# skyzh/tiny-llm

Hardware: AMD Instinct MI355X
Metric: Qwen3-4B int4 decode tokens/sec/GPU; achieved HBM GB/s vs roofline (higher is better)
Workload: dtype bf16; 1 GPU; Qwen3-4B int4 single-prompt KV-cache decode (BASELINE.json configs[1]); decode_steps=2003, batch_per_gpu=1, parallelism=request-parallel x1 (no collective on the data path), page_size=128, graph_replay=True, prefill_step=128, replay_route=aql

## Files before the change

include/tinyllm_engine.h:

```cpp
#ifndef TINYLLM_ENGINE_H
#define TINYLLM_ENGINE_H

#include <stddef.h>
#include <stdint.h>

#ifdef __cplusplus
extern "C" {
#endif

typedef struct tl_engine tl_engine;

typedef struct tl_w4 {
    const uint32_t *weight_dev;
    const void *scales_dev;
    const void *biases_dev;
    int rows;
    int cols;
} tl_w4;

typedef struct tl_layer_weights {
    tl_w4 wqkv, wo, wgu, wdown;
    const void *input_norm_dev;
    const void *post_norm_dev;
    const void *q_norm_dev;
    const void *k_norm_dev;
} tl_layer_weights;

typedef struct tl_engine_config {
    int hidden_size, num_layers, num_heads, num_kv_heads, head_dim, intermediate_size, vocab_size;
    float rope_theta, rms_norm_eps;
    int page_size;
    int num_pages;
    int max_batch;
    int max_pages_per_seq;
    int max_prefill_rows;
} tl_engine_config;

typedef struct tl_engine_stats {
    int pages_in_use, pages_free, peak_pages_in_use;
    long page_allocations, reused_page_allocations;
    long decode_steps, graph_captures, graph_replays, prefill_tokens;
    size_t kv_bytes, workspace_bytes;
    long graph_cache_flushes;
    long aql_steps;
} tl_engine_stats;

typedef struct tl_moe_weights {
    tl_w4 router;
    const uint32_t *gate_dev, *up_dev, *down_dev;
    const void *gate_scales_dev, *gate_biases_dev, *up_scales_dev, *up_biases_dev, *down_scales_dev, *down_biases_dev;
    int num_experts;
    int experts_per_token;
    int intermediate_size;
    int norm_topk_prob;
} tl_moe_weights;

int tl_engine_create(const tl_engine_config *cfg, const tl_layer_weights *layers, const tl_w4 *embed,
                     const void *final_norm_dev, const tl_w4 *lm_head, void *stream, tl_engine **out);
enum { TL_KV_BF16 = 0, TL_KV_FP8_E4M3 = 1 };
int tl_engine_create_kv(const tl_engine_config *cfg, const tl_layer_weights *layers, const tl_w4 *embed, const void *final_norm_dev,
                        const tl_w4 *lm_head, void *stream, int kv_format, tl_engine **out);
int tl_engine_kv_format(const tl_engine *e);
int tl_engine_set_moe_layer(tl_engine *e, int layer, const tl_moe_weights *w);
int tl_engine_set_option(tl_engine *e, const char *name, int value);
void tl_engine_destroy(tl_engine *e);
int tl_engine_synchronize(tl_engine *e);

int tl_engine_begin(tl_engine *e, int slot);
int tl_engine_reserve(tl_engine *e, int slot, int total_tokens);
int tl_engine_release(tl_engine *e, int slot);
int tl_engine_rewind(tl_engine *e, int slot, int n);
int tl_engine_context_len(const tl_engine *e, int slot);
int tl_engine_move(tl_engine *e, int src, int dst);

int tl_engine_prefill(tl_engine *e, int slot, const int32_t *tokens, int n, int want_logits);

int tl_engine_prefill_packed(tl_engine *e, int n_seqs, const int *slots, const int32_t *tokens, const int *lens,
                             const int *want_logits);

int tl_engine_fork(tl_engine *e, int src, int dst);

typedef struct tl_prefix_stats {
    long lookups, hits, tokens_matched, tail_rows_copied, pages_registered, pages_evicted;
    int entries, pages_retained, max_retained_pages, enabled;
} tl_prefix_stats;
int tl_engine_prefix_cache(tl_engine *e, int enabled, int max_retained_pages);
int tl_engine_prefix_attach(tl_engine *e, int slot, const int32_t *tokens, int n, int *matched);
int tl_engine_prefix_extend(tl_engine *e, int slot, const int32_t *tokens, int n);
int tl_engine_prefix_clear(tl_engine *e);
int tl_engine_prefix_stats(const tl_engine *e, tl_prefix_stats *out);
typedef struct tl_kv_pool_desc {
    void *base_dev;
    size_t row_bytes;
} tl_kv_pool_desc;
int tl_kv_copy_rows(const tl_kv_pool_desc *pools_dev, int n_pools, int heads, int page_size, int from_page, int to_page, int rows,
                    void *stream);

typedef struct tl_swap_stats {
    int host_pages, host_pages_in_use;
    long parks, unparks, pages_out, pages_in;
    size_t record_bytes;
} tl_swap_stats;
int tl_engine_swap_space(tl_engine *e, int host_pages);
int tl_engine_park(tl_engine *e, int slot);
int tl_engine_unpark(tl_engine *e, int slot);
int tl_engine_slot_parked(const tl_engine *e, int slot);
int tl_engine_step_pages(const tl_engine *e, int batch, int *need, int *obtainable);
int tl_engine_swap_stats(const tl_engine *e, tl_swap_stats *out);
size_t tl_kv_page_record_bytes(const tl_kv_pool_desc *pools_host, int n_pools, int heads, int page_size);
int tl_kv_gather_pages(const tl_kv_pool_desc *pools_dev, const size_t *record_offsets_dev, int n_pools, int heads, int page_size,
                       const int32_t *page_ids_dev, int n_pages, int tail_rows, void *staging_dev, size_t record_bytes, void *stream);
int tl_kv_scatter_pages(const tl_kv_pool_desc *pools_dev, const size_t *record_offsets_dev, int n_pools, int heads, int page_size,
                        const int32_t *page_ids_dev, int n_pages, int tail_rows, const void *staging_dev, size_t record_bytes, void *stream);

int tl_engine_verify(tl_engine *e, int slot, const int32_t *tokens, int n, int32_t *out_ids);

int tl_engine_verify_sampled(tl_engine *e, int slot, const int32_t *tokens, int n, const void *draft_logits_dev, float draft_temperature,
// ... 157 lines not shown
    int launches;
    int rows_per_pass;
    int p[5];
} tl_linear_info;

size_t tl_decode_linear_workspace_bytes(int M, int rows, int cols);
int tl_decode_linear(const tl_tiled_w4 *w, const void *a_dev, void *out_dev, int M, int prologue, int epilogue,
                     const void *norm_w_dev, const void *residual_dev, float eps, int kernel, void *workspace_dev,
                     size_t workspace_bytes, void *stream, tl_linear_info *info);

typedef struct tl_linear_ex {
    const float *merge_ws_dev;
    int n_splits;
    const float *ss_in_dev;
    int ss_in_n;
    float *ss_out_dev;
    const void *norm_out_dev;
    void *out_w_dev;
    int fragment_order;
} tl_linear_ex;
int tl_decode_linear_ex(const tl_tiled_w4 *w, const void *a_dev, void *out_dev, int M, int prologue, int epilogue,
                        const void *norm_w_dev, const void *residual_dev, float eps, int kernel, void *workspace_dev,
                        size_t workspace_bytes, void *stream, const tl_linear_ex *ex, tl_linear_info *info);

int tl_prefill_weights_bf16(const tl_w4 *w, void *out_dev, void *stream);
int tl_prefill_matmul_bf16(const void *a_dev, const void *w_bf16_dev, void *out_dev, int M, int rows, int cols, int epilogue,
                           const void *residual_dev, void *stream);

int tl_decode_gemv_plan(int M, int rows, int cols, int *out5);
int tl_decode_gemv_variant_compiled(int MR, int KS, int CW, int LM);
int tl_decode_batched_plan(int M, int rows, int cols, int *out6);
int tl_decode_batched_variant_compiled(int MB, int GPW);
int tl_decode_streaming_plan(int M, int rows, int cols, int *out4);
int tl_decode_streaming_variant_compiled(int T, int GPW);
int tl_decode_attention_plan(int batch, int max_context, int num_heads, int num_kv_heads, int *out3);

typedef struct tl_attention_info {
    int n_splits, tokens_per_split, heads_per_workgroup;
    int launches;
} tl_attention_info;
size_t tl_decode_attention_fused_workspace_bytes(int batch, int num_heads, int head_dim);
int tl_decode_attention_fused(const void *qkv_dev, const void *q_norm_dev, const void *k_norm_dev, void *key_pages_dev,
                              void *value_pages_dev, const int32_t *block_table_dev, const int32_t *context_lens_dev,
                              void *out_dev, int batch, int num_heads, int num_kv_heads, int head_dim, int page_size,
                              int max_pages, float rope_theta, float eps, int max_context, void *workspace_dev,
                              size_t workspace_bytes, void *stream, tl_attention_info *info);
int tl_decode_attention_fused_fp8(const void *qkv_dev, const void *q_norm_dev, const void *k_norm_dev, void *key_pages_dev,
                                  float *key_scales_dev, void *value_pages_dev, float *value_scales_dev,
                                  const int32_t *block_table_dev, const int32_t *context_lens_dev, void *out_dev, int batch,
                                  int num_heads, int num_kv_heads, int head_dim, int page_size, int max_pages, float rope_theta,
                                  float eps, int max_context, void *workspace_dev, size_t workspace_bytes, void *stream,
                                  tl_attention_info *info);

int tl_sample_logits(const void *logits_dev, int rows, int vocab, const float *temperature_dev, const int32_t *top_k_dev,
                     const float *top_p_dev, const uint64_t *seed_dev, const int32_t *position_dev, int32_t *ids_dev, void *stream);

int tl_spec_sample_rows(const void *target_logits_dev, const void *draft_logits_dev, int rows, int vocab, const int32_t *proposal_dev,
                        const float *temperature_dev, const int32_t *top_k_dev, const float *top_p_dev, const float *draft_temperature_dev,
                        const int32_t *draft_top_k_dev, const float *draft_top_p_dev, const uint64_t *seed_dev, const int32_t *position_dev,
                        int32_t *accept_dev, int32_t *alt_dev, void *stream);

int tl_logprob_rows(const void *logits_dev, int rows, int vocab, const int32_t *ids_dev, int top_n, float *logprob_dev, int32_t *top_ids_dev,
                    float *top_logprobs_dev, void *stream);

int tl_pool_rows(const void *rows_dev, int hidden, int n_seqs, const int *row0, const int *len, const int *finish, const int *prior, int pooling,
                 float *sums_dev, int normalize, int dim, float *out_dev, void *stream);

int tl_truncate_rows(const void *logits_dev, int rows, int vocab, const float *temperature_dev, const float *min_p_dev, const float *typical_p_dev,
                     const float *mu_dev, void *out_dev, float *kept_logsum_dev, void *stream);
int tl_mirostat_update_rows(const void *filtered_dev, int rows, int vocab, const int32_t *ids_dev, const float *temperature_dev,
                            const float *kept_logsum_dev, const float *tau_dev, const float *eta_dev, float *mu_dev, void *stream);

int tl_process_logits(const void *logits_dev, int rows, int vocab, const uint16_t *history_dev, const float *repetition_dev,
                      const float *presence_dev, const float *frequency_dev, const int32_t *bias_ids_dev, const float *bias_values_dev,
                      const int32_t *bias_n_dev, void *out_dev, void *stream);

int tl_verify_attention_rows(const void *qkv_dev, const void *q_norm_dev, const void *k_norm_dev, void *key_pages_dev, void *value_pages_dev,
                             float *key_scales_dev, float *value_scales_dev, const int32_t *block_table_dev, int n_seqs, const int *slots,
                             const int *starts, const int *lens, void *out_dev, int num_heads, int num_kv_heads, int page_size, int max_pages,
                             float rope_theta, float eps, void *stream, tl_attention_info *info);
int tl_verify_accept_rows(const void *logits_dev, int vocab, int n_seqs, const int *row0, const int *lens, const int32_t *tokens_dev,
                          tl_verify_result *out_dev, void *stream);

#ifdef __cplusplus
}
#endif
#endif
```

include/tinyllm_hip.h:

```cpp
#ifndef TINYLLM_HIP_H
#define TINYLLM_HIP_H

#include <stddef.h>
#include <stdint.h>

#ifdef __cplusplus
extern "C" {
#endif

typedef enum tl_dtype {
    TL_F32 = 0,
    TL_F16 = 1,
    TL_BF16 = 2,
} tl_dtype;

typedef enum tl_status {
    TL_OK = 0,
    TL_ERR_INVALID = -1,
    TL_ERR_UNSUPPORTED = -2,
    TL_ERR_HIP = -3,
} tl_status;

const char *tl_last_error(void);

int tl_abi_version(void);

int tl_load_library(const char *path);

int tl_quantized_matmul(const void *scales, const void *biases, const void *a, const uint32_t *b, void *out, int M,
                        int N, int K, int group_size, int bits, tl_dtype dtype, int use_simdgroup, int use_split_k,
                        void *workspace, size_t workspace_bytes, void *stream);
size_t tl_quantized_matmul_workspace_bytes(int M, int N, int K, tl_dtype dtype, int use_simdgroup, int use_split_k);
int tl_quantized_matmul_split_k(int M, int N, int K, int use_simdgroup, int use_split_k);

int tl_quantized_embedding(const void *indices, int indices_unsigned, const void *scales, const void *biases,
                           const uint32_t *weight, void *out, int tokens, int dim, int vocab, int group_size, int bits,
                           tl_dtype dtype, void *stream);

int tl_rms_norm(const void *x, const void *weight, void *out, int rows, int dim, float eps, tl_dtype dtype,
                void *stream);

int tl_rope(const void *x, const int32_t *offsets, void *out, int B, int L, int H, int D, int dims, float base,
            int traditional, tl_dtype dtype, void *stream);

int tl_swiglu(const void *gate, const void *up, void *out, size_t size, tl_dtype dtype, void *stream);

int tl_decode_attention(const void *q, const void *k, const void *v, const float *mask, void *out, int q_rows, int L,
                        int S, int D, int num_heads, int num_kv_heads, float scale, int is_causal, int has_mask,
                        tl_dtype dtype, void *stream);

int tl_gather_quantized_matvec(const void *scales, const void *biases, const void *a, const uint32_t *b,
                               const int32_t *expert_ids, void *out, int M, int N, int K, int num_experts,
                               int group_size, int bits, tl_dtype dtype, void *stream);

int tl_paged_cache_update(void *pages, const void *values, int num_pages, int heads, int page_size, int head_dim,
                          int length, int page_id, int start, tl_dtype dtype, void *stream);

int tl_paged_attention(const void *q, const void *key_pages, const void *value_pages, const int32_t *block_table,
                       const int32_t *context_lens, void *out, int N, int L, int D, int num_pages, int page_size,
                       int max_pages, int num_heads, int num_kv_heads, float scale, int is_causal,
                       int max_context_hint, tl_dtype dtype, void *workspace, size_t workspace_bytes, void *stream);
size_t tl_paged_attention_workspace_bytes(int N, int L, int D, int page_size, int max_pages, int num_heads,
                                          int num_kv_heads, int max_context_hint);
int tl_paged_attention_waves(int waves);

int tl_kv_fp8_quantize_rows(const void *values, void *codes, float *scales, long rows, int head_dim, void *stream);
int tl_kv_fp8_dequantize_rows(const void *codes, const float *scales, void *out, long rows, int head_dim, void *stream);
int tl_paged_cache_update_fp8(void *pages, float *page_scales, const void *values, int num_pages, int heads, int page_size,
                              int head_dim, int length, int page_id, int start, void *stream);
int tl_paged_attention_fp8(const void *q, const void *key_pages, const float *key_scales, const void *value_pages,
                           const float *value_scales, const int32_t *block_table, const int32_t *context_lens, void *out, int N,
                           int L, int D, int num_pages, int page_size, int max_pages, int num_heads, int num_kv_heads, float scale,
                           int is_causal, int max_context_hint, void *workspace, size_t workspace_bytes, void *stream);


#ifdef __cplusplus
}
#endif
#endif
```

tiny-llm_amd/csrc/attention.hip:

```cpp
#include <type_traits>

#include "common.h"
#include "kv8.h"

namespace tl {

constexpr float LOG2E = 1.44269504089f;

template <typename TT>
__global__ __launch_bounds__(256) void decode_attention_kernel(const typename TT::storage *__restrict__ q,
                                                               const typename TT::storage *__restrict__ k,
                                                               const typename TT::storage *__restrict__ v,
                                                               const float *__restrict__ mask,
                                                               typename TT::storage *__restrict__ out, int q_rows,
                                                               int L, int S, int D, int num_heads, int num_kv_heads,
                                                               float scale, int is_causal, int has_mask) {
    constexpr int MAXV = 16;
    extern __shared__ __attribute__((aligned(16))) float dsm[];
    const int query_index = blockIdx.x;
    const int query_row = query_index / L;
    const int qp = query_index - query_row * L;
    const int batch = query_row / num_heads;
    const int qh = query_row - batch * num_heads;
    const int kvh = qh / (num_heads / num_kv_heads);
// ... 74 lines not shown
    const long within = idx - rowi * vec_per_row;
    const int head = (int)(rowi / length);
    const int token = (int)(rowi - (long)head * length);
    const long dst = (((long)page_id * heads + head) * page_size + start + token) * row_bytes + within * BYTES;
    const long src = rowi * row_bytes + within * BYTES;
    if constexpr (BYTES == 16) {
        *reinterpret_cast<uint4 *>(pages + dst) = *reinterpret_cast<const uint4 *>(values + src);
    } else if constexpr (BYTES == 4) {
        *reinterpret_cast<uint32_t *>(pages + dst) = *reinterpret_cast<const uint32_t *>(values + src);
    } else {
        *reinterpret_cast<uint16_t *>(pages + dst) = *reinterpret_cast<const uint16_t *>(values + src);
    }
}

__global__ __launch_bounds__(256) void kv8_quantize_rows_kernel(const uint16_t *__restrict__ values, uint8_t *__restrict__ pages,
                                                                float *__restrict__ scales, long rows, int length, int page_size,
                                                                long page_row0, int start) {
    const long row = (long)blockIdx.x * 16 + (threadIdx.x >> 4);
    const int t = threadIdx.x & 15;
    const long r = min(row, rows - 1);
    const u32x4 raw = *reinterpret_cast<const u32x4 *>(values + r * 128 + t * 8);
    float x[8];
#pragma unroll
    for (int i = 0; i < 4; ++i) {
        x[2 * i] = __uint_as_float(raw[i] << 16);
        x[2 * i + 1] = __uint_as_float(raw[i] & 0xffff0000u);
    }
    u32x2 codes;
    float sc, deq[8];
    kv8_quantize_row16(x, codes, sc, deq);
    if (row >= rows) return;
    const long h = r / length, tt = r - h * length;
    const long dst = page_row0 + h * page_size + start + tt;
    *reinterpret_cast<u32x2 *>(pages + dst * 128 + t * 8) = codes;
    if (t == 0) scales[dst] = sc;
}

__global__ __launch_bounds__(256) void kv8_dequantize_rows_kernel(const uint8_t *__restrict__ codes, const float *__restrict__ scales,
                                                                  uint16_t *__restrict__ out, long rows) {
    const long i = (long)blockIdx.x * 256 + threadIdx.x;
    if (i >= rows * 16) return;
    const u32x2 c = *reinterpret_cast<const u32x2 *>(codes + i * 8);
    *reinterpret_cast<u32x4 *>(out + i * 8) = kv8_to_bf16x8(c, scales[i >> 4]);
}

constexpr int PD_RQ = 4;

template <typename TT, int VD, bool VEC, bool KV8 = false>
__global__ __launch_bounds__(256) void paged_decode_kernel(
    const typename TT::storage *__restrict__ q, const typename TT::storage *__restrict__ key_pages,
    const typename TT::storage *__restrict__ value_pages, const int32_t *__restrict__ block_table,
    const int32_t *__restrict__ context_lens, typename TT::storage *__restrict__ out, float *__restrict__ ws, int L,
    int D, int page_size, int max_pages, int num_heads, int num_kv_heads, float scale, int is_causal, int n_splits,
    int n_row_chunks, const float *__restrict__ key_scales = nullptr, const float *__restrict__ value_scales = nullptr) {
    static_assert(!KV8 || (VD == 8 && VEC), "FP8 pages: head dimension 128");
    using S = typename TT::storage;
    extern __shared__ __attribute__((aligned(16))) float psm[];
    const int split = blockIdx.x % n_splits;
    const int chunk = blockIdx.x / n_splits;
    const int kvh = blockIdx.y;
    const int b = blockIdx.z;
    const int rep = num_heads / num_kv_heads;
    const int R = rep * L;
    const int g = threadIdx.x >> 4;
    const int t = threadIdx.x & 15;
    const int ctx = context_lens[b];
    const float scale_log2 = scale * LOG2E;
    const int stride = D + 2;

    int rq_n[PD_RQ], rq_qp[PD_RQ], rq_vis[PD_RQ];
    bool rq_ok[PD_RQ];
    float qv[PD_RQ][VD], acc[PD_RQ][VD], m[PD_RQ], l[PD_RQ];
    int max_vis = 0;
#pragma unroll
    for (int r = 0; r < PD_RQ; ++r) {
        const int rr = chunk * PD_RQ + r;
        rq_ok[r] = rr < R;
        const int hq = rq_ok[r] ? rr / L : 0;
        rq_qp[r] = rq_ok[r] ? rr - hq * L : 0;
        rq_n[r] = b * num_heads + kvh * rep + hq;
        int vis = is_causal ? min(max(ctx - L + rq_qp[r] + 1, 0), ctx) : ctx;
        rq_vis[r] = rq_ok[r] ? vis : 0;
        max_vis = max(max_vis, rq_vis[r]);
        m[r] = -1e30f;
        l[r] = 0.f;
        const S *qp = q + ((long)rq_n[r] * L + rq_qp[r]) * D;
#pragma unroll
        for (int i = 0; i < VD; ++i) {
            const int d = VEC ? t * VD + i : t + 16 * i;
            qv[r][i] = (rq_ok[r] && d < D) ? TT::to_float(qp[d]) * scale_log2 : 0.f;
            acc[r][i] = 0.f;
        }
    }
    const int per = ((max_vis + n_splits - 1) / n_splits + 15) & ~15;
    const int t_begin = split * per;
    const int t_end = min(t_begin + per, max_vis);

    for (int tok = t_begin + g; tok < t_end; tok += 16) {
        const int lp = tok / page_size;
        const int slot = tok - lp * page_size;
        const int page_id = lp < max_pages ? block_table[(long)b * max_pages + lp] : -1;
        if (page_id < 0) continue;
        const long off = (((long)page_id * num_kv_heads + kvh) * page_size + slot) * D;
        float kf[VD], vf[VD];
        float k_s = 1.f, v_s = 1.f;
        if constexpr (KV8) {
            const u32x2 kc = *reinterpret_cast<const u32x2 *>(reinterpret_cast<const uint8_t *>(key_pages) + off + t * VD);
// ... 31 lines not shown
            }
        }
#pragma unroll
        for (int r = 0; r < PD_RQ; ++r) {
            float part = 0.f;
#pragma unroll
            for (int i = 0; i < VD; ++i) part += qv[r][i] * kf[i];
            const float score = KV8 ? group16_sum(part) * k_s : group16_sum(part);
            if (tok < rq_vis[r]) {
                const float nm = fmaxf(m[r], score);
                const float of = exp2_hw(m[r] - nm);
                const float sf = exp2_hw(score - nm);
                l[r] = l[r] * of + sf;
                const float sfv = KV8 ? sf * v_s : sf;
#pragma unroll
                for (int i = 0; i < VD; ++i) acc[r][i] = acc[r][i] * of + sfv * vf[i];
                m[r] = nm;
            }
        }
    }

#pragma unroll
    for (int r = 0; r < PD_RQ; ++r) {
        float *dst = psm + ((long)g * PD_RQ + r) * stride;
#pragma unroll
        for (int i = 0; i < VD; ++i) {
            const int d = VEC ? t * VD + i : t + 16 * i;
            if (d < D) dst[d] = acc[r][i];
        }
        if (t == 0) {
            dst[D] = m[r];
            dst[D + 1] = l[r];
        }
    }
    __syncthreads();
    for (int item = threadIdx.x; item < PD_RQ * D; item += 256) {
        const int r = item / D;
        const int d = item - r * D;
        const int rr = chunk * PD_RQ + r;
        if (rr >= R) continue;
        const int hq_o = rr / L;
        const int qp_o = rr - hq_o * L;
        float gm = -1e30f;
#pragma unroll
        for (int j = 0; j < 16; ++j) gm = fmaxf(gm, psm[((long)j * PD_RQ + r) * stride + D]);
        float gl = 0.f, vs = 0.f;
#pragma unroll
        for (int j = 0; j < 16; ++j) {
            const float *src = psm + ((long)j * PD_RQ + r) * stride;
            const float f = exp2_hw(src[D] - gm);
            gl += src[D + 1] * f;
            vs += src[d] * f;
        }
        const long orow = ((long)b * num_heads + kvh * rep + hq_o) * L + qp_o;
        if (n_splits == 1) {
            out[orow * D + d] = TT::from_float(gl == 0.f ? 0.f : vs / gl);
        } else {
            float *w = ws + (orow * n_splits + split) * stride;
            w[d] = vs;
            if (d == 0) {
                w[D] = gm;
                w[D + 1] = gl;
            }
        }
    }
}

template <typename TT>
__global__ __launch_bounds__(128) void paged_merge_kernel(const float *__restrict__ ws,
                                                          typename TT::storage *__restrict__ out, int D,
                                                          int n_splits) {
    const long orow = blockIdx.x;
    const int stride = D + 2;
    const float *base = ws + orow * n_splits * stride;
    float gm = -1e30f;
    for (int s = 0; s < n_splits; ++s) gm = fmaxf(gm, base[s * stride + D]);
    for (int d = threadIdx.x; d < D; d += blockDim.x) {
        float gl = 0.f, vs = 0.f;
        for (int s = 0; s < n_splits; ++s) {
            const float f = exp2_hw(base[s * stride + D] - gm);
            gl += base[s * stride + D + 1] * f;
            vs += base[s * stride + d] * f;
        }
        out[orow * D + d] = TT::from_float(gl == 0.f ? 0.f : vs / gl);
    }
}

#ifndef FA_ABL
#define FA_ABL 0
#endif
constexpr int FA_BK = 64;
constexpr int FA_SUB = FA_BK / 32;
constexpr int FA_VROW = 128 + 32;

__device__ __forceinline__ void fa_sload_i32(const int32_t *ptr, int &dst) { asm volatile("s_load_dword %0, %1, 0x0" : "=s"(dst) : "s"(ptr)); }
__device__ __forceinline__ void fa_sload_wait(int &a) { asm volatile("s_waitcnt lgkmcnt(0)" : "+s"(a)); }
constexpr int FA_KS_ELEMS = FA_BK * 128, FA_VS_ELEMS = FA_BK * FA_VROW;
constexpr size_t fa_pipe_lds_bytes() { return (size_t)2 * (FA_KS_ELEMS + FA_VS_ELEMS) * 2 + 2 * FA_BK * sizeof(int); }
template <bool ONEPAGE, int QR = 1, bool KV8 = false, int NW = 4>
__global__ __launch_bounds__(64 * NW, (QR == 1 && NW == 4) ? 2 : 1) void paged_fa_bf16_d128_kernel(
    const uint16_t *__restrict__ q, const void *__restrict__ key_pages_v, const void *__restrict__ value_pages_v,
    const int32_t *__restrict__ block_table, const int32_t *__restrict__ context_lens, uint16_t *__restrict__ out,
    float *__restrict__ ws, int n_splits, int L, int page_size, int page_shift, int max_pages, int num_heads, int num_kv_heads,
    float scale, int is_causal, int xcd_remap, const float *__restrict__ key_scales = nullptr,
    const float *__restrict__ value_scales = nullptr) {
    constexpr int D = 128;
    using KVE = typename std::conditional<KV8, uint8_t, uint16_t>::type;
    using KVC = typename std::conditional<KV8, u32x2, u32x4>::type;
    const KVE *__restrict__ key_pages = reinterpret_cast<const KVE *>(key_pages_v);
    const KVE *__restrict__ value_pages = reinterpret_cast<const KVE *>(value_pages_v);
    constexpr bool PIPE = NW == 8;
    static_assert(NW == 4 || (NW == 8 && ONEPAGE && QR == 1), "8 waves: pages of 64+ tokens, one row block per wave");
    constexpr int NT = 64 * NW;
    constexpr int CPT = FA_BK * 16 / NT;
    extern __shared__ __attribute__((aligned(16))) unsigned char fa_dyn[];
    __shared__ __attribute__((aligned(16))) uint16_t ks_one[PIPE ? 8 : FA_KS_ELEMS];
    __shared__ __attribute__((aligned(16))) uint16_t vs_one[PIPE ? 8 : FA_VS_ELEMS];
    __shared__ int tile_page_one[PIPE ? 2 : 2 * FA_BK];
    uint16_t *const ks = PIPE ? reinterpret_cast<uint16_t *>(fa_dyn) : ks_one;
    uint16_t *const vs = PIPE ? reinterpret_cast<uint16_t *>(fa_dyn) + 2 * FA_KS_ELEMS : vs_one;
    int *const tile_page = PIPE ? reinterpret_cast<int *>(fa_dyn + (size_t)2 * (FA_KS_ELEMS + FA_VS_ELEMS) * 2) : tile_page_one;

    const int tid = threadIdx.x;
    const int wave = tid >> 6;
    const int lane = tid & 63;
    const int l32 = lane & 31;
    const int h = lane >> 5;
    int bx = blockIdx.x, kvh = blockIdx.y;
    if (xcd_remap) {
        const int gx = gridDim.x, T = gx * (int)gridDim.y;
        const int l = blockIdx.x + gx * blockIdx.y;
        const int c = l & 7;
        const int t = c * (T >> 3) + min(c, T & 7) + (l >> 3);
        kvh = t / gx;
        bx = t - kvh * gx;
    }
    const int b = blockIdx.z;
    const int rep = num_heads / num_kv_heads;
    const int QB = (L + 32 * QR - 1) / (32 * QR);
    const int items = rep * QB;
    const int split = bx % n_splits;
    const int item_block = is_causal ? ((int)gridDim.x / n_splits - 1 - bx / n_splits) : bx / n_splits;
    const int item = item_block * NW + wave;
    const bool wave_live = item < items;
    const int hq = wave_live ? item % rep : 0;
    const int qb = wave_live ? item / rep : 0;
    const int n = b * num_heads + kvh * rep + hq;
    const int ctx = context_lens[b];
    const float scale_log2 = scale * LOG2E;
    int qrow[QR];
    bool q_valid[QR];
    u32x4 qf[QR][8];
    f32x16 o[QR][4];
    float run_max[QR], run_sum[QR];
#pragma unroll
    for (int rb = 0; rb < QR; ++rb) {
        qrow[rb] = (qb * QR + rb) * 32 + l32;
        q_valid[rb] = wave_live && qrow[rb] < L;
// ... 282 lines not shown
        for (int stage = stage_begin; stage < stage_end; ++stage) {
            __syncthreads();
            if (!(FA_ABL & 8) || stage == stage_begin) stage_store(sa, 0, stage & 1);
            __syncthreads();
            if (stage + 1 < stage_end && !(FA_ABL & 16)) {
                stage_load(stage + 1, sa);
                if (stage + 2 < stage_end) load_pids(stage + 2);
            }
            compute_stage(stage, 0, stage & 1);
        }
    } else if (stage_begin < stage_end) {
        const int32_t *brow = block_table + (long)b * max_pages;
        const int last = stage_end - 1;
        auto page_slot = [&](int stage) { return brow + min((stage * FA_BK) >> page_shift, max_pages - 1); };
        auto page_live = [&](int stage, int id) { return ((stage * FA_BK) >> page_shift) < max_pages ? id : -1; };
        int pg0, pg1, pg_n;
        fa_sload_i32(page_slot(stage_begin), pg0);
        fa_sload_i32(page_slot(min(stage_begin + 1, last)), pg1);
        fa_sload_i32(page_slot(min(stage_begin + 2, last)), pg_n);
        fa_sload_wait(pg0);
        fa_sload_wait(pg1);
        fa_sload_wait(pg_n);
        stage_load(stage_begin, sa, page_live(stage_begin, pg0));
        stage_store(sa, 0, 0);
        stage_load(min(stage_begin + 1, last), sa, page_live(min(stage_begin + 1, last), pg1));
        for (int stage = stage_begin, r = 0; stage < stage_end; ++stage, ++r) {
            __syncthreads();
            if (stage + 1 < stage_end && !(FA_ABL & 8)) stage_store(sa, (r + 1) & 1, (r + 1) & 1);
            const int s2 = min(stage + 2, last);
            if (!(FA_ABL & 16)) stage_load(s2, sa, page_live(s2, pg_n));
            fa_sload_i32(page_slot(min(stage + 3, last)), pg_n);
            compute_stage(stage, r & 1, r & 1);
            fa_sload_wait(pg_n);
        }
    }

#pragma unroll
    for (int rb = 0; rb < QR; ++rb) {
        if (!q_valid[rb]) continue;
        if (n_splits > 1) {
            float *w = ws + (((long)n * L + qrow[rb]) * n_splits + split) * (D + 2);
#pragma unroll
            for (int db = 0; db < 4; ++db)
#pragma unroll
                for (int rg = 0; rg < 4; ++rg)
#pragma unroll
                    for (int e = 0; e < 4; ++e) w[db * 32 + 8 * rg + 4 * h + e] = o[rb][db][4 * rg + e];
            if (h == 0) {
                w[D] = run_max[rb] == -INFINITY ? -1e30f : run_max[rb];
                w[D + 1] = run_sum[rb];
            }
            continue;
        }
        uint16_t *orow = out + ((long)n * L + qrow[rb]) * D;
        const float inv = run_sum[rb] == 0.f ? 0.f : 1.0f / run_sum[rb];
#pragma unroll
        for (int db = 0; db < 4; ++db) {
#pragma unroll
            for (int rg = 0; rg < 4; ++rg) {
                u32x2 pk;
                pk[0] = BF16::pack2(o[rb][db][4 * rg + 0] * inv, o[rb][db][4 * rg + 1] * inv);
                pk[1] = BF16::pack2(o[rb][db][4 * rg + 2] * inv, o[rb][db][4 * rg + 3] * inv);
                *reinterpret_cast<u32x2 *>(orow + db * 32 + 8 * rg + 4 * h) = pk;
            }
        }
    }
}

static int pick_fa_splits(int B, int Hkv, int item_blocks, int max_ctx, int wg_target = 512) {
    const int base = std::max(1, B * Hkv * item_blocks);
    int s = wg_target / base;
    s = std::min(s, std::max(1, max_ctx / 256));
    s = std::min(s, 32);
    return std::max(s, 1);
}

static int pick_splits(int B, int Hkv, int row_chunks, int max_ctx) {
    const int base = std::max(1, B * Hkv * row_chunks);
    int s = (512 + base - 1) / base;
    const int by_len = std::max(1, max_ctx / 64);
    s = std::min(s, by_len);
    s = std::min(s, 64);
    return std::max(s, 1);
}
int paged_decode_splits(int B, int Hkv, int row_chunks, int max_ctx) { return pick_splits(B, Hkv, row_chunks, max_ctx); }

}

using namespace tl;

extern "C" int tl_decode_attention(const void *q, const void *k, const void *v, const float *mask, void *out,
                                   int q_rows, int L, int S, int D, int num_heads, int num_kv_heads, float scale,
                                   int is_causal, int has_mask, tl_dtype dtype, void *stream) {
    TL_REQUIRE(q && k && v && out, "decode_attention: null pointer");
    TL_REQUIRE(D > 0 && D <= 256 && num_heads > 0 && num_kv_heads > 0 && num_heads % num_kv_heads == 0 &&
                   q_rows % num_heads == 0,
               "decode_attention: incompatible attention shapes");
    TL_REQUIRE(!has_mask || mask, "decode_attention: mask must have shape [B*Hq,L,S]");
    if (q_rows == 0 || L == 0) return TL_OK;
    hipStream_t st = (hipStream_t)stream;
    const size_t lds = (size_t)(16 * D + 32) * sizeof(float);
    const dim3 grid(q_rows * L), block(256);
#define DA_LAUNCH(TT)                                                                                            \
    hipLaunchKernelGGL((decode_attention_kernel<TT>), grid, block, lds, st, (const typename TT::storage *)q,     \
                       (const typename TT::storage *)k, (const typename TT::storage *)v, mask,                   \
                       (typename TT::storage *)out, q_rows, L, S, D, num_heads, num_kv_heads, scale, is_causal, \
                       has_mask)
// ... 15 lines not shown
    TL_REQUIRE(pages && values, "paged_cache_update: null pointer");
    TL_REQUIRE(heads > 0 && page_size > 0 && head_dim > 0 && length >= 0,
               "paged_cache_update: expected pages [P, H, page_size, D] and values [1, H, length, D]");
    TL_REQUIRE(page_id >= 0 && page_id < num_pages && start >= 0 && start + length <= page_size,
               "paged_cache_update: destination slice is outside page storage");
    if (length == 0) return TL_OK;
    hipStream_t st = (hipStream_t)stream;
    const long esz = dtype == TL_F32 ? 4 : 2;
    const long row_bytes = (long)head_dim * esz;
    const bool a16 = row_bytes % 16 == 0 && ((uintptr_t)pages % 16 == 0) && ((uintptr_t)values % 16 == 0);
    if (a16) {
        const long total = (long)heads * length * (row_bytes / 16);
        hipLaunchKernelGGL((paged_cache_update_kernel<16>), dim3(ceil_div(total, 256)), dim3(256), 0, st,
                           (const char *)values, (char *)pages, heads, length, row_bytes, page_size, page_id, start);
    } else if (esz == 4) {
        const long total = (long)heads * length * (row_bytes / 4);
        hipLaunchKernelGGL((paged_cache_update_kernel<4>), dim3(ceil_div(total, 256)), dim3(256), 0, st,
                           (const char *)values, (char *)pages, heads, length, row_bytes, page_size, page_id, start);
    } else {
        const long total = (long)heads * length * (row_bytes / 2);
        hipLaunchKernelGGL((paged_cache_update_kernel<2>), dim3(ceil_div(total, 256)), dim3(256), 0, st,
                           (const char *)values, (char *)pages, heads, length, row_bytes, page_size, page_id, start);
    }
    TL_CHECK_LAUNCH("paged_cache_update");
    return TL_OK;
}

static bool paged_uses_fa(int L, int D, tl_dtype dtype) { return L > 8 && dtype == TL_BF16 && D == 128; }
static int g_fa_waves = 8;
extern "C" int tl_paged_attention_waves(int waves) {
    const int before = g_fa_waves;
    if (waves == 4 || waves == 8) g_fa_waves = waves;
    return before;
}

extern "C" size_t tl_paged_attention_workspace_bytes(int N, int L, int D, int page_size, int max_pages, int num_heads,
                                                     int num_kv_heads, int max_context_hint) {
    if (N <= 0 || L <= 0 || num_heads <= 0 || num_kv_heads <= 0) return 0;
    const int B = N / num_heads;
    const int rep = num_heads / num_kv_heads;
    const int row_chunks = (rep * L + PD_RQ - 1) / PD_RQ;
    const int max_ctx = max_context_hint > 0 ? max_context_hint : max_pages * page_size;
    int splits = pick_splits(B, num_kv_heads, row_chunks, max_ctx);
    if (L > 8 && D == 128)
        splits = std::max(splits, pick_fa_splits(B, num_kv_heads, (rep * ((L + 31) / 32) + 3) / 4, max_ctx));
    if (splits <= 1) return 0;
    return (size_t)N * L * splits * (D + 2) * sizeof(float);
}

static int paged_attention_impl(const void *q, const void *key_pages, const void *value_pages, const float *key_scales,
                                const float *value_scales, const int32_t *block_table, const int32_t *context_lens, void *out, int N,
                                int L, int D, int num_pages, int page_size, int max_pages, int num_heads, int num_kv_heads, float scale,
                                int is_causal, int max_context_hint, tl_dtype dtype, void *workspace, size_t workspace_bytes,
                                void *stream) {
    const bool kv8 = key_scales != nullptr;
    TL_REQUIRE(dtype == TL_F32 || dtype == TL_BF16,
               "paged_attention: q, key_pages, and value_pages must have the same float32 or bfloat16 dtype");
    TL_REQUIRE(q && key_pages && value_pages && block_table && context_lens && out, "paged_attention: null pointer");
    TL_REQUIRE(num_heads > 0 && num_kv_heads > 0 && num_heads % num_kv_heads == 0,
               "paged_attention: num_heads must be divisible by num_kv_heads");
    TL_REQUIRE(N % num_heads == 0, "paged_attention: q.shape[0] must be divisible by num_heads");
    TL_REQUIRE(page_size > 0 && max_pages > 0 && num_pages > 0 && L > 0,
               "paged_attention: page tensors must be 4D [P, H_kv, page_size, D]");
    TL_REQUIRE(D > 0 && D <= 128, "paged_attention: head dimension must be at most 128");
    if (N == 0) return TL_OK;
    hipStream_t st = (hipStream_t)stream;
    const int B = N / num_heads;
    const int rep = num_heads / num_kv_heads;

    if (L > 8 && dtype == TL_BF16) {
        if (D != 128) return fail(TL_ERR_UNSUPPORTED, "paged_attention: bfloat16 prefill requires head dimension 128");
        TL_REQUIRE(scale > 0.f, "paged_attention: the bfloat16 FlashAttention path needs a positive scale");
        constexpr int qr = 1;
        const int items = rep * ((L + 32 * qr - 1) / (32 * qr));
        int page_shift = -1;
        for (int sh = 0; sh < 30; ++sh)
            if ((1 << sh) == page_size) page_shift = sh;
        const bool w8 = g_fa_waves == 8 && page_shift >= 6 && L >= 64;
        const int nw = w8 ? 8 : 4;
        const int item_blocks = (items + nw - 1) / nw;
        const int max_ctx_fa = max_context_hint > 0 ? max_context_hint : max_pages * page_size;
        int fa_splits = pick_fa_splits(B, num_kv_heads, item_blocks, max_ctx_fa, w8 ? 256 : 512);
        const size_t fa_need = fa_splits > 1 ? (size_t)N * L * fa_splits * (D + 2) * sizeof(float) : 0;
        if (fa_need > 0 && (!workspace || workspace_bytes < fa_need)) fa_splits = 1;
        const dim3 grid(item_blocks * fa_splits, num_kv_heads, B);
        const int fa_xcd_remap = 1;
#define FA_LAUNCH(ONEP, QRv, K8)                                                                                                \
        hipLaunchKernelGGL((paged_fa_bf16_d128_kernel<ONEP, QRv, K8>), grid, dim3(256), 0, st, (const uint16_t *)q, key_pages,  \
                           value_pages, block_table, context_lens, (uint16_t *)out, (float *)workspace, fa_splits, L, page_size, \
                           page_shift, max_pages, num_heads, num_kv_heads, scale, is_causal, fa_xcd_remap, key_scales,            \
                           value_scales)
#define FA_LAUNCH8(K8)                                                                                                           \
        do {                                                                                                                         \
            static bool attr_set_dev[64] = {};        \
            int dev_ = 0;                                                                                                            \
            (void)hipGetDevice(&dev_);                                                                                               \
            bool &attr_set = attr_set_dev[dev_ & 63];                                                                                \
            if (!attr_set) {                                                                                                         \
                if (hipFuncSetAttribute(reinterpret_cast<const void *>(&paged_fa_bf16_d128_kernel<true, 1, K8, 8>),                  \
                                        hipFuncAttributeMaxDynamicSharedMemorySize, (int)fa_pipe_lds_bytes()) != hipSuccess)         \
                    return fail(TL_ERR_HIP, "paged_attention: cannot size the prefill kernel's LDS");                               \
                attr_set = true;                                                                                                     \
            }                                                                                                                        \
            hipLaunchKernelGGL((paged_fa_bf16_d128_kernel<true, 1, K8, 8>), grid, dim3(512), fa_pipe_lds_bytes(), st,                \
                               (const uint16_t *)q, key_pages, value_pages, block_table, context_lens, (uint16_t *)out,             \
                               (float *)workspace, fa_splits, L, page_size, page_shift, max_pages, num_heads, num_kv_heads, scale,   \
                               is_causal, fa_xcd_remap, key_scales, value_scales);                                                   \
        } while (0)
        if (w8) {
            if (kv8) FA_LAUNCH8(true);
            else FA_LAUNCH8(false);
        } else if (kv8) {
            if (page_shift >= 6) FA_LAUNCH(true, 1, true);
            else FA_LAUNCH(false, 1, true);
        } else if (page_shift >= 6) FA_LAUNCH(true, 1, false);
        else FA_LAUNCH(false, 1, false);
#undef FA_LAUNCH
#undef FA_LAUNCH8
        TL_CHECK_LAUNCH("paged_attention(prefill)");
        if (fa_splits > 1) {
            hipLaunchKernelGGL((paged_merge_kernel<BF16>), dim3(N * L), dim3(128), 0, st, (const float *)workspace,
                               (uint16_t *)out, D, fa_splits);
            TL_CHECK_LAUNCH("paged_attention(prefill merge)");
        }
        return TL_OK;
    }

    const int row_chunks = (rep * L + PD_RQ - 1) / PD_RQ;
    const int max_ctx = max_context_hint > 0 ? max_context_hint : max_pages * page_size;
    const int splits = pick_splits(B, num_kv_heads, row_chunks, max_ctx);
    const size_t need = splits > 1 ? (size_t)N * L * splits * (D + 2) * sizeof(float) : 0;
    if (need > 0 && (!workspace || workspace_bytes < need))
        return fail(TL_ERR_INVALID, "paged_attention: workspace is missing or too small");
    const dim3 grid(splits * row_chunks, num_kv_heads, B), block(256);
    const size_t lds = (size_t)16 * PD_RQ * (D + 2) * sizeof(float);
    float *ws = (float *)workspace;
#define PD_LAUNCH(TT, VDv, VECv)                                                                                    \
    hipLaunchKernelGGL((paged_decode_kernel<TT, VDv, VECv>), grid, block, lds, st, (const typename TT::storage *)q, \
                       (const typename TT::storage *)key_pages, (const typename TT::storage *)value_pages,         \
                       block_table, context_lens, (typename TT::storage *)out, ws, L, D, page_size, max_pages,     \
                       num_heads, num_kv_heads, scale, is_causal, splits, row_chunks)
    if (kv8) {
        hipLaunchKernelGGL((paged_decode_kernel<BF16, 8, true, true>), grid, block, lds, st, (const uint16_t *)q,
                           (const uint16_t *)key_pages, (const uint16_t *)value_pages, block_table, context_lens, (uint16_t *)out, ws,
                           L, D, page_size, max_pages, num_heads, num_kv_heads, scale, is_causal, splits, row_chunks, key_scales,
                           value_scales);
    } else if (dtype == TL_BF16) {
        if (D == 128) PD_LAUNCH(BF16, 8, true);
        else if (D == 64) PD_LAUNCH(BF16, 4, true);
        else PD_LAUNCH(BF16, 8, false);
    } else {
        if (D == 128) PD_LAUNCH(F32, 8, true);
        else if (D == 64) PD_LAUNCH(F32, 4, true);
        else PD_LAUNCH(F32, 8, false);
    }
#undef PD_LAUNCH
    TL_CHECK_LAUNCH("paged_attention(decode)");
    if (splits > 1) {
        if (dtype == TL_BF16) {
            hipLaunchKernelGGL((paged_merge_kernel<BF16>), dim3(N * L), dim3(128), 0, st, ws, (uint16_t *)out, D, splits);
        } else {
            hipLaunchKernelGGL((paged_merge_kernel<F32>), dim3(N * L), dim3(128), 0, st, ws, (float *)out, D, splits);
        }
        TL_CHECK_LAUNCH("paged_attention(merge)");
    }
    (void)paged_uses_fa;
    return TL_OK;
}

extern "C" int tl_paged_attention(const void *q, const void *key_pages, const void *value_pages,
                                  const int32_t *block_table, const int32_t *context_lens, void *out, int N, int L,
                                  int D, int num_pages, int page_size, int max_pages, int num_heads, int num_kv_heads,
                                  float scale, int is_causal, int max_context_hint, tl_dtype dtype, void *workspace,
                                  size_t workspace_bytes, void *stream) {
    return paged_attention_impl(q, key_pages, value_pages, nullptr, nullptr, block_table, context_lens, out, N, L, D, num_pages, page_size,
                                max_pages, num_heads, num_kv_heads, scale, is_causal, max_context_hint, dtype, workspace, workspace_bytes,
                                stream);
}

extern "C" int tl_kv_fp8_quantize_rows(const void *values, void *codes, float *scales, long rows, int head_dim, void *stream) {
    TL_REQUIRE(values && codes && scales, "kv_fp8_quantize_rows: null pointer");
    TL_REQUIRE(head_dim == 128 && rows >= 0 && rows < (1L << 30), "kv_fp8_quantize_rows: fewer than 2^30 rows of 128 bfloat16 values");
    if (rows == 0) return TL_OK;
    hipLaunchKernelGGL(kv8_quantize_rows_kernel, dim3(ceil_div(rows, 16)), dim3(256), 0, (hipStream_t)stream, (const uint16_t *)values,
                       (uint8_t *)codes, scales, rows, (int)rows, (int)rows, 0L, 0);
    TL_CHECK_LAUNCH("kv_fp8_quantize_rows");
    return TL_OK;
}

extern "C" int tl_kv_fp8_dequantize_rows(const void *codes, const float *scales, void *out, long rows, int head_dim, void *stream) {
    TL_REQUIRE(codes && scales && out, "kv_fp8_dequantize_rows: null pointer");
    TL_REQUIRE(head_dim == 128 && rows >= 0, "kv_fp8_dequantize_rows: rows of 128 codes");
    if (rows == 0) return TL_OK;
    hipLaunchKernelGGL(kv8_dequantize_rows_kernel, dim3(ceil_div(rows * 16, 256)), dim3(256), 0, (hipStream_t)stream,
                       (const uint8_t *)codes, scales, (uint16_t *)out, rows);
    TL_CHECK_LAUNCH("kv_fp8_dequantize_rows");
    return TL_OK;
}

extern "C" int tl_paged_cache_update_fp8(void *pages, float *page_scales, const void *values, int num_pages, int heads, int page_size,
                                         int head_dim, int length, int page_id, int start, void *stream) {
    TL_REQUIRE(pages && page_scales && values, "paged_cache_update_fp8: null pointer");
    TL_REQUIRE(head_dim == 128, "paged_cache_update_fp8: FP8 pages need head dimension 128");
    TL_REQUIRE(heads > 0 && page_size > 0 && length >= 0,
               "paged_cache_update_fp8: expected pages [P, H, page_size, 128] and bfloat16 values [1, H, length, 128]");
    TL_REQUIRE(page_id >= 0 && page_id < num_pages && start >= 0 && start + length <= page_size,
               "paged_cache_update_fp8: destination slice is outside page storage");
    if (length == 0) return TL_OK;
    const long rows = (long)heads * length;
    hipLaunchKernelGGL(kv8_quantize_rows_kernel, dim3(ceil_div(rows, 16)), dim3(256), 0, (hipStream_t)stream, (const uint16_t *)values,
                       (uint8_t *)pages, page_scales, rows, length, page_size, (long)page_id * heads * page_size, start);
    TL_CHECK_LAUNCH("paged_cache_update_fp8");
    return TL_OK;
}

extern "C" int tl_paged_attention_fp8(const void *q, const void *key_pages, const float *key_scales, const void *value_pages,
                                      const float *value_scales, const int32_t *block_table, const int32_t *context_lens, void *out,
                                      int N, int L, int D, int num_pages, int page_size, int max_pages, int num_heads, int num_kv_heads,
                                      float scale, int is_causal, int max_context_hint, void *workspace, size_t workspace_bytes,
                                      void *stream) {
    TL_REQUIRE(key_scales && value_scales, "paged_attention_fp8: null scale pointer");
    TL_REQUIRE(D == 128, "paged_attention_fp8: FP8 pages need head dimension 128");
    return paged_attention_impl(q, key_pages, value_pages, key_scales, value_scales, block_table, context_lens, out, N, L, D, num_pages,
                                page_size, max_pages, num_heads, num_kv_heads, scale, is_causal, max_context_hint, TL_BF16, workspace,
                                workspace_bytes, stream);
}
```

tiny-llm_amd/csrc/decode_linear.h:

```cpp
#pragma once

#include <algorithm>
#include <cstdlib>
#include <initializer_list>
#include <map>
#include <memory>
#include <string>
#include <vector>

#include "../../include/tinyllm_engine.h"
#include "common.h"
#include "device_block.h"
#include "engine_kernels.h"
#include "qmv.h"
#include "qmv3.h"
#include "qmm3.h"
#include "qmm6.h"
#include "qmm7.h"
#include "gemm8.h"

namespace tl {

#define TL_TRY(expr)                  \
    do {                              \
// ... 183 lines not shown
            a3.residual = args.residual;
            a3.eps = args.eps;
            a3.M = args.M;
            a3.N = args.N;
            a3.K = args.K;
            a3.prof = args.prof;
            if (ctx.gemv_producer_ss) {
                if ((p.pro == PRO_RMSNORM || p.pro == PRO_RMS_WEIGHTED) && p.ss_in && p.ss_in_n > 0)
                    a3.ss_in = p.ss_in + (size_t)m0 * p.ss_in_n, a3.ss_n = p.ss_in_n;
                if (p.epi == EPI_RESIDUAL && p.ss_out) a3.ss_out = p.ss_out + (size_t)m0 * (w.rows / 16);
            }
            if (p.tile_max && p.epi == EPI_STORE && step == M && w.rows % 16 == 0) {
                a3.tile_max = p.tile_max;
                r.maxima_rows = M;
            }
            if (p.out_w) {
                TL_REQUIRE(p.epi == EPI_RESIDUAL && p.norm_out && step == M, "engine: weighted rows need the residual epilogue and one pass");
                a3.norm_out = (const uint16_t *)p.norm_out;
                a3.out_w = p.out_w;
            }
            if ((merge ? launch_qmv3_attn_merge_bf16(a3, p.n_splits, ctx.stream) : launch_qmv3_bf16(a3, p.pro, p.epi, ctx.stream)) != 0)
                return fail(TL_ERR_UNSUPPORTED, merge ? "engine: no wo GEMV that merges the attention partials for this shape" : "engine: MFMA GEMV launch failed");
            if (pc) prof_after(pc, p.kind, p3.blocks);
            report_launch(ctx, 1, 1, step, {p3.MR, p3.KS, p3.CW, p3.LM, p3.blocks});
            continue;
        }
        all_emitted = false;
        TL_REQUIRE(p.out_w == nullptr && p.pro != PRO_RMS_WEIGHTED && !merge, "engine: weighted rows are a route of the MFMA GEMV only");
        if (launch_qmv_fused_bf16(args, p.pro, p.epi, ctx.stream) != 0)
            return fail(TL_ERR_UNSUPPORTED, "engine: no GEMV configuration for this shape");
        if (pc) prof_after(pc, p.kind, qmv_plan(args.M, args.N, args.K).blocks);
        report_launch(ctx, 3, 1, step);
    }
    TL_CHECK_LAUNCH(merge ? "engine wo gemv with merge" : "engine gemv");
    if (all_emitted && w.rows % 16 == 0) r.ss_n = w.rows / 16;
    return TL_OK;
}

static int ensure_splitk(const LinearCtx &ctx, size_t bytes) {
    if (bytes <= ctx.splitk_ws_bytes) return TL_OK;
    return fail(TL_ERR_INVALID, "engine: matmul workspace too small for this shape (sized at tl_engine_create: " +
                                    std::to_string(ctx.splitk_ws_bytes) + " bytes, need " + std::to_string(bytes) + ")");
}

static int engine_qmm(LinearCtx &ctx, const tl_w4 &w, const uint16_t *a, uint16_t *out, int M) {
    const size_t need = tl_quantized_matmul_workspace_bytes(M, w.cols, w.rows, TL_BF16, 1, 1);
    TL_TRY(ensure_splitk(ctx, need));
    return tl_quantized_matmul(w.scales_dev, w.biases_dev, a, w.weight_dev, out, M, w.cols, w.rows, 128, 4, TL_BF16, 1, 1,
                               ctx.splitk_ws, ctx.splitk_ws_bytes, ctx.stream);
}

constexpr int GEMM8_MIN_ROWS = 1792;
static bool gemm8_wins(int M) { return M >= GEMM8_MIN_ROWS; }
static int engine_gemm(LinearCtx &ctx, const Proj &p, bool *norm_done = nullptr) {
    const tl_w4 &w = *p.w;
    const int M = p.M;
    if (norm_done) *norm_done = false;
    if (ctx.use_gemm8 && gemm8_wins(M)) {
        const auto wb = ctx.bf16w.find(w.weight_dev);
        if (wb != ctx.bf16w.end() && gemm8_applicable(M, w.rows, w.cols)) {
            Gemm8Args g{};
            g.a = p.a, g.w = wb->second, g.out = p.out, g.residual = p.residual, g.M = M, g.N = w.rows, g.K = w.cols;
            if (launch_gemm8_bf16(g, p.epi, ctx.stream) != 0) return fail(TL_ERR_UNSUPPORTED, "engine: bf16 GEMM launch failed");
            TL_CHECK_LAUNCH("engine bf16 matmul");
            return TL_OK;
        }
    }
    if (p.epi != EPI_STORE && M > 8 && ctx.gemm_fused_epilogue) {
        const size_t need = tl_quantized_matmul_workspace_bytes(M, w.cols, w.rows, TL_BF16, 1, 1);
        TL_TRY(ensure_splitk(ctx, need));
        TL_TRY(qmm_bf16_epilogue(w.scales_dev, w.biases_dev, p.a, w.weight_dev, p.out, M, w.cols, w.rows, p.epi, p.residual, ctx.splitk_ws,
                                 ctx.splitk_ws_bytes, ctx.stream, ctx.fuse_reduce_norm ? (const uint16_t *)p.norm_out : nullptr, p.out_w,
                                 ctx.rms_norm_eps, norm_done));
        TL_CHECK_LAUNCH("engine matmul");
        return TL_OK;
    }
    uint16_t *plain = p.epi == EPI_STORE ? p.out : (p.epi == EPI_SWIGLU ? ctx.gu : ctx.tmp);
    TL_TRY(engine_qmm(ctx, w, p.a, plain, M));
    if (p.epi == EPI_SWIGLU) {
        const long n4 = (long)M * (w.rows / 2) / 4;
        hipLaunchKernelGGL(swiglu_interleaved_kernel, dim3(ceil_div(n4, 256)), dim3(256), 0, ctx.stream, plain, p.out, n4);
    } else if (p.epi == EPI_RESIDUAL) {
        const long n8 = (long)M * w.rows / 8;
        hipLaunchKernelGGL(residual_add_kernel, dim3(ceil_div(n8, 256)), dim3(256), 0, ctx.stream, p.residual, plain, p.out, n8);
    }
    TL_CHECK_LAUNCH("engine matmul");
    return TL_OK;
}

static bool qmm6_takes(const LinearCtx &ctx, const tl_w4 &w, int M) {
    return ctx.use_qmm6 && ctx.force_linear == 0 && M >= ctx.qmm3_min_rows && M <= 64 && ctx.tiled.count(w.weight_dev) != 0 &&
           qmm6_plan(M, w.cols, w.rows).ok;
}
static int engine_qmm6(LinearCtx &ctx, const Proj &p, ProfCtx *pc = nullptr, ProjResult *res = nullptr) {
    ProjResult none, &r = res ? *res : none;
    r = ProjResult{};
    const tl_w4 &w = *p.w;
    const int M = p.M;
    const auto tiled = ctx.tiled.find(w.weight_dev);
    TL_REQUIRE(tiled != ctx.tiled.end(), "engine: the register-resident matmul needs the tiled weights");
    const bool a_frag = p.frag && p.ss_in != nullptr && p.epi != EPI_RESIDUAL;
    const Qmm7Plan p7 = (ctx.use_qmm7 || ctx.force_qmm7) && a_frag && p.out_w == nullptr ? qmm7_plan(M, w.cols, w.rows) : Qmm7Plan{};
    TL_REQUIRE(p7.ok || !ctx.force_qmm7, "engine: the row-streaming matmul takes weighted rows in fragment order (store / SwiGLU) at the shapes of qmm7_plan");
    const Qmm6Plan pl = qmm6_plan(M, w.cols, w.rows, a_frag);
    TL_REQUIRE(p7.ok || pl.ok, "engine: the register-resident matmul does not cover this shape");
    Qmm6Args q{};
    q.wt = tiled->second.wt;
    q.sbt = tiled->second.sbt;
    q.a = p.a;
    q.out = p.out;
    q.residual = p.residual;
    q.norm_out = (const uint16_t *)p.norm_out;
    q.out_w = p.out_w;
    q.ss = p.ss_in;
    q.ss_n = p.ss_in ? p.ss_in_n : 0;
    q.ss_out = p.epi == EPI_RESIDUAL ? p.ss_out : nullptr;
    q.eps = ctx.rms_norm_eps;
    q.M = M;
    q.N = w.cols;
    q.K = w.rows;
    q.prof = pc ? pc->buf : nullptr;
    q.a_frag = a_frag;
    q.out_w_frag = (p.out_w_frag >= 0 ? p.out_w_frag != 0 : p.frag) && p.out_w != nullptr;
    int n_wg = 0;
    if (p7.ok) {
        if (launch_qmm7_bf16(q, p.epi, ctx.stream, &n_wg) != 0) return fail(TL_ERR_UNSUPPORTED, "engine: row-streaming matmul launch failed");
        if (pc) prof_after(pc, p.kind, n_wg);
        report_launch(ctx, 6, 1, p7.MB * 16, {p7.MB, p7.GPW, p7.T, p7.row_blocks, n_wg});
        TL_CHECK_LAUNCH("engine row-streaming matmul");
        return TL_OK;
// ... 271 lines not shown
```

tiny-llm_amd/csrc/engine.hip:

```cpp
#include <dlfcn.h>

#include <cstddef>
#include <cstring>
#include <memory>

#include "decode_linear.h"
#include "device_block.h"
#include "step_end.h"
#include "logit_process.h"
#include "truncate.h"
#include "grammar_stack.h"
#include "attn_mfma.h"
#include "aql.h"
#include "prefix_cache.h"
#include "kv_copy.h"
#include "beam.h"
#include "kv_swap.h"
#include "pool.h"
#include "lora.h"
#include "slot_settings.h"
#include "slot_table.h"
#include "stop.h"
#include "stop_set.h"
#include "verify_attn_host.h"
// ... 48 lines not shown
            }
        }
        return c;
    }
};

struct tl_stop {
    StopSet set;
    const tl_vocab *vocab = nullptr;
    DeviceBlock mem;
    StopDev *dev = nullptr;
};

struct tl_engine {
    tl_engine_config cfg{};
    std::vector<tl_layer_weights> layers;
    tl_w4 embed{}, lm_head{};
    const void *final_norm = nullptr;
    hipStream_t stream = nullptr;
    struct OwnedStream {
        hipStream_t s = nullptr;
        ~OwnedStream() {
            if (s) (void)hipStreamDestroy(s);
        }
    } owned_stream;

    DeviceBlock arena;
    size_t arena_bytes = 0;
    DeviceBlock kv_mem[4];
    uint16_t *kpool = nullptr, *vpool = nullptr;
    size_t layer_pool_elems = 0, kv_bytes = 0;
    int kv_format = TL_KV_BF16;
    float *kscale_pool = nullptr, *vscale_pool = nullptr;
    size_t layer_scale_elems = 0;
    size_t kv_elem_bytes() const { return kv_format == TL_KV_FP8_E4M3 ? 1 : 2; }
    float *layer_ks(int l) const { return kscale_pool ? kscale_pool + (size_t)l * layer_scale_elems : nullptr; }
    float *layer_vs(int l) const { return vscale_pool ? vscale_pool + (size_t)l * layer_scale_elems : nullptr; }
    LinearCtx lin;
    std::vector<TiledW4Mem> tiled_mem;
    std::vector<DeviceBlock> bf16w_mem;
    DeviceBlock splitk_mem;
    size_t tiled_bytes = 0, bf16w_bytes = 0;

    int32_t *block_table = nullptr, *context_lens = nullptr, *tokens = nullptr, *live = nullptr, *produced = nullptr,
            *ring = nullptr, *scratch_ctx = nullptr, *prefill_tokens = nullptr;
    uint16_t *x = nullptr, *h = nullptr, *xn = nullptr, *qkv = nullptr, *q_t = nullptr, *attn_t = nullptr,
             *attn = nullptr, *act = nullptr, *logits = nullptr;
    float *attn_ws = nullptr;
    int last_attn_launches = 0;
    f32x2 *lm_tile_max = nullptr;
    bool lm_tile_max_on = true;
    float *ss_x = nullptr, *ss_h = nullptr;
    bool attn_qkv_partials = true;
    bool wo_merges_attn = true;
    int32_t *verify_ids = nullptr;
    struct SpecRecord {
        int32_t proposal[8];
        float t_temperature[8];
        int32_t t_top_k[8];
        float t_top_p[8], d_temperature[8];
        int32_t d_top_k[8];
        float d_top_p[8];
        int32_t position[8];
        uint64_t seed[8];
        int32_t accept[8], alt[8];
    };
    DeviceBlock spec_mem;
    SpecRecord *spec_rec = nullptr;
    int attn_rq = 0;
    int attn_rq1_ctx = 4096;
    int attn_rq1_batch = 2;
    int attn_min_tokens = 64;
    int attn_wg_cap = 0;
    bool attn_min_tokens_auto = true;
    bool attn_mfma = true;
    int attn_max_splits = 64;
    int attn_max_splits_gqa = 32;
    size_t attn_ws_bytes = 0;
    int rows_cap = 0;
    int ring_cap = 4096;

    SlotTable table;
    SlotEdits step_edits;
    DeviceBlock kv_pools_mem;
    tl_kv_pool_desc *kv_pools_dev = nullptr;
    int kv_pools_n = 0;
    std::vector<tl_kv_pool_desc> kv_pools_host;
    DeviceBlock swap_host, swap_staging;
    DeviceBlock swap_offsets_mem;
    size_t *swap_offsets_dev = nullptr;
    size_t swap_record_bytes = 0;
    int swap_staging_pages = 0;
    long swap_parks = 0, swap_unparks = 0, swap_pages_out = 0, swap_pages_in = 0;
    bool slot_runs(int slot) const { return table.runs(slot); }
    tl_engine_stats stats{};
    SlotSettings settings;
    DeviceBlock settings_mem[SB_COUNT];
    template <class T>
    T *sdev(int block, size_t off) const {
        return block == SB_LORA ? (T *)((char *)lora_slot_dev + off) : settings_mem[block].at<T>(off);
    }
    const tl_grammar *grammar_of(int slot) const { return (const tl_grammar *)settings.slots[slot].pen.grammar.id; }
    DeviceBlock score_mem;
    uint16_t *score_logits = nullptr;
    int32_t *score_ids = nullptr, *score_argmax = nullptr;
    float *score_lp = nullptr;
// ... 1086 lines not shown
    return TL_OK;
}

extern "C" int tl_engine_set_moe_layer(tl_engine *e, int layer, const tl_moe_weights *w) {
    TL_REQUIRE(e && w, "engine_set_moe_layer: null argument");
    const tl_engine_config &c = e->cfg;
    TL_REQUIRE(layer >= 0 && layer < c.num_layers, "engine_set_moe_layer: layer out of range");
    TL_REQUIRE(e->plans.empty() && e->stats.decode_steps == 0 && e->stats.prefill_tokens == 0,
               "engine_set_moe_layer: call it before the first prefill / decode");
    TL_REQUIRE(w->num_experts > 0 && w->num_experts <= 1024 && w->experts_per_token > 0 && w->experts_per_token <= 16 &&
                   w->experts_per_token <= w->num_experts,
               "engine_set_moe_layer: need 1 <= experts_per_token <= min(16, num_experts) and num_experts <= 1024");
    TL_REQUIRE(w->intermediate_size > 0 && w->intermediate_size % 128 == 0, "engine_set_moe_layer: intermediate_size must be a positive multiple of 128");
    TL_TRY(check_w4(w->router, w->num_experts, c.hidden_size, "moe router"));
    TL_REQUIRE(w->gate_dev && w->up_dev && w->down_dev && w->gate_scales_dev && w->gate_biases_dev && w->up_scales_dev &&
                   w->up_biases_dev && w->down_scales_dev && w->down_biases_dev,
               "engine_set_moe_layer: null expert tensor");
    TL_REQUIRE((long)e->rows_cap * w->experts_per_token <= 65535, "engine_set_moe_layer: max_prefill_rows x experts_per_token must stay below 65536 (one grouped launch)");
    for (int M : {1, 8, 9, e->rows_cap})
        TL_REQUIRE(tl_quantized_matmul_workspace_bytes(std::min(M, e->rows_cap), c.hidden_size, w->num_experts, TL_BF16, 1, 1) <= e->lin.splitk_ws_bytes,
                   "engine_set_moe_layer: the router matmul does not fit the engine's matmul workspace");
    const int k = std::max(e->moe_k_max, w->experts_per_token), E = std::max(e->moe_e_max, w->num_experts),
              I = std::max(e->moe_i_max, w->intermediate_size);
    if (k != e->moe_k_max || E != e->moe_e_max || I != e->moe_i_max) {
        const size_t R = (size_t)e->rows_cap;
        Carve carve;
        const size_t o_log = carve(R * E * 2), o_ids = carve(R * k * 4), o_sc = carve(R * k * 2), o_g = carve(R * k * I * 2),
                     o_u = carve(R * k * I * 2), o_a = carve(R * k * I * 2), o_y = carve(R * k * c.hidden_size * 2);
        TL_HIP(hipStreamSynchronize(e->stream));
        TL_TRY(e->moe_ws.alloc(carve.off, "hipMalloc((void **)&e->moe_ws, carve.off): " + std::string(hipGetErrorString(hipErrorOutOfMemory))));
        e->moe_ws_bytes = carve.off;
        char *A = e->moe_ws.at();
        e->moe_logits = (uint16_t *)(A + o_log);
        e->moe_ids = (int32_t *)(A + o_ids);
        e->moe_scores = (uint16_t *)(A + o_sc);
        e->moe_gate = (uint16_t *)(A + o_g);
        e->moe_up = (uint16_t *)(A + o_u);
        e->moe_act = (uint16_t *)(A + o_a);
        e->moe_y = (uint16_t *)(A + o_y);
        e->moe_k_max = k, e->moe_e_max = E, e->moe_i_max = I;
        e->stats.workspace_bytes = e->arena_bytes + e->tiled_bytes + e->moe_ws_bytes;
    }
    e->moe[layer] = *w;
    if (e->layer_act_mem) {
        TL_HIP(hipStreamSynchronize(e->stream));
        e->layer_act_mem.reset();
        e->layer_act.clear();
        e->layer_act_rows = 0, e->layer_act_bytes = 0, e->layer_ws_bytes = 0;
        e->layer_plane_bytes[0] = e->layer_plane_bytes[1] = 0;
    }
    return TL_OK;
}

extern "C" int tl_engine_set_option(tl_engine *e, const char *name, int value) {
    TL_REQUIRE(e && name, "engine_set_option: null argument");
    TL_REQUIRE(e->plans.empty() && e->stats.decode_steps == 0 && e->stats.prefill_tokens == 0,
               "engine_set_option: call it before the first prefill / decode (captured steps hold the routes they were captured with)");
    const std::string n = name;
    const bool on = value != 0;
    if (n == "qmm3") e->lin.use_qmm3 = on;
    else if (n == "qmm6") e->lin.use_qmm6 = on;
    else if (n == "qmm7") e->lin.use_qmm7 = on;
    else if (n == "attn_qkv_partials") e->attn_qkv_partials = on;
    else if (n == "lmhead_tile_max") e->lm_tile_max_on = on;
    else if (n == "gemm_fused_epilogue") e->lin.gemm_fused_epilogue = on;
    else if (n == "gemm8") e->lin.use_gemm8 = on;
    else if (n == "prefill_reduce_norm") e->lin.fuse_reduce_norm = on;
    else if (n == "aql_fences") e->aql_fences.inner_acquire = e->aql_fences.inner_release = on ? HSA_FENCE_SCOPE_AGENT : HSA_FENCE_SCOPE_NONE;
    else return fail(TL_ERR_INVALID, "engine_set_option: unknown option '" + n + "' (qmm3, qmm6, qmm7, gemm8, prefill_reduce_norm, attn_qkv_partials, lmhead_tile_max, gemm_fused_epilogue, aql_fences)");
    return TL_OK;
}

static void drop_plans(tl_engine *e) {
    for (auto &kv : e->plans) (void)hipGraphExecDestroy(kv.second.exec);
    e->plans.clear();
}

extern "C" void tl_engine_destroy(tl_engine *e) {
    if (!e) return;
    (void)aql_drain(e);
    (void)hipStreamSynchronize(e->stream);
    drop_plans(e);
    delete e;
}

extern "C" int tl_engine_kv_format(const tl_engine *e) { return e ? e->kv_format : TL_KV_BF16; }

extern "C" const char *tl_engine_replay_route(const tl_engine *e) {
    static thread_local std::string text;
    if (!e) return "";
    text = e->aql_on ? std::string("aql") : ("hipgraph" + (e->aql_why.empty() ? std::string() : ": " + e->aql_why));
    const char *why = e->aql_on ? graph_only_reason(step_features(e, 0, e->cfg.max_batch)) : nullptr;
    if (why) text = std::string("hipgraph: ") + why;
    return text.c_str();
}

extern "C" int tl_engine_synchronize(tl_engine *e) {
    TL_REQUIRE(e, "engine_synchronize: null engine");
    TL_HIP(hipStreamSynchronize(e->stream));
    return TL_OK;
}

extern "C" int tl_engine_begin(tl_engine *e, int slot) {
    TL_REQUIRE(e, "engine: null engine");
    TL_TRY(table_rc(e->table.begin(slot)));
    Pokes pk;
    pk.emplace_back(e->live + slot, 1);
    pk.emplace_back(e->context_lens + slot, 0);
    pk.emplace_back(e->produced + slot, 0);
    pk.emplace_back(e->tokens + slot, 0);
    SettingsEdits sed;
    e->settings.reset(slot, sed);
    return settings_apply(e, sed, pk);
}

extern "C" int tl_engine_reserve(tl_engine *e, int slot, int total_tokens) {
    TL_TRY(slot_check_unparked(e, slot));
    TL_REQUIRE(total_tokens >= 0, "engine_reserve: total_tokens must be nonnegative");
    SlotEdits ed;
    Pokes pk;
    TL_TRY(table_rc(e->table.reserve(slot, total_tokens, ed)));
    TL_TRY(apply_edits(e, ed, pk));
    return poke(e, pk);
// ... 960 lines not shown
    std::vector<LoraDesc> descs(n_adapters, LoraDesc{});
    for (int i = 0; i < n_adapters; ++i) {
        const tl_lora_matrices &m = adapters[i];
        LoraDesc &d = descs[i];
        TL_REQUIRE(m.a_dev && m.b_dev && (uintptr_t)m.a_dev % 16 == 0 && (uintptr_t)m.b_dev % 16 == 0, "lora_rows: adapter matrices must be 16-byte aligned");
        TL_REQUIRE(m.rank >= 8 && m.rank <= TL_MAX_LORA_RANK && m.rank % 8 == 0, "lora_rows: rank must be a multiple of 8 up to 64");
        TL_REQUIRE(std::isfinite(m.scale), "lora_rows: scale must be finite");
        TL_REQUIRE(m.seg_mask > 0 && m.seg_mask < (1 << n_seg), "lora_rows: seg_mask names no segment, or one the layout does not have");
        d.a = (const uint16_t *)m.a_dev, d.b = (const uint16_t *)m.b_dev, d.scale = m.scale, d.rank = m.rank;
        for (int s = 0; s < 3; ++s) {
            d.t_off[s] = -1;
            if (s < n_seg && ((m.seg_mask >> s) & 1)) d.t_off[s] = d.rtot, d.rtot += m.rank;
        }
    }
    std::vector<LoraTile> tiles;
    bool looks_up = n_tiles == 0;
    if (n_tiles == 0) lora_lookup_tiles(rows, tiles);
    else {
        TL_REQUIRE(n_tiles > 0 && tile_row0 && tile_rows && tile_adapter, "lora_rows: a tile list needs its three arrays");
        for (int i = 0; i < n_tiles; ++i) {
            TL_REQUIRE(tile_row0[i] >= 0 && tile_rows[i] >= 0 && tile_rows[i] <= LORA_TILE && (long)tile_row0[i] + tile_rows[i] <= rows,
                       "lora_rows: a tile is up to 16 rows inside [0, rows)");
            TL_REQUIRE(tile_adapter[i] >= LORA_ROW_LOOKUP && tile_adapter[i] < n_adapters, "lora_rows: a tile's adapter is -2 (per row), -1 (none) or an index");
            looks_up = looks_up || tile_adapter[i] == LORA_ROW_LOOKUP;
            tiles.push_back(LoraTile{tile_row0[i], tile_rows[i], tile_adapter[i], 0});
        }
    }
    TL_REQUIRE(!looks_up || row_adapter_dev, "lora_rows: tiles that look their rows' adapters up need row_adapter_dev");
    const int nt = (int)tiles.size();
    Carve carve;
    const size_t o_table = carve(descs.size() * sizeof(LoraDesc)), o_tiles = carve(tiles.size() * sizeof(LoraTile));
    const size_t o_part = carve(lora_partial_floats(nt, std::max(in, 1)) * 4), o_ss = carve(lora_ss_floats(nt, std::max(in, 1)) * 4);
    DeviceBlock ws;
    TL_TRY(ws.alloc(carve.off, "lora_rows: hipMalloc(workspace) failed"));
    char *const mem = ws.at();
    int rc = TL_OK;
    if (hipMemcpy(mem + o_table, descs.data(), descs.size() * sizeof(LoraDesc), hipMemcpyHostToDevice) != hipSuccess ||
        hipMemcpy(mem + o_tiles, tiles.data(), tiles.size() * sizeof(LoraTile), hipMemcpyHostToDevice) != hipSuccess)
        rc = fail(TL_ERR_HIP, "lora_rows: hipMemcpy(table) failed");
    if (rc == TL_OK) {
        LoraCall c;
        c.table = (const LoraDesc *)(mem + o_table), c.stride = 1, c.index = 0, c.n_adapters = n_adapters, c.row_adapter = row_adapter_dev;
        c.tiles_dev = (const LoraTile *)(mem + o_tiles), c.n_tiles = nt, c.total_rows = rows, c.x = (const uint16_t *)x_dev, c.in = in, c.out = out;
        c.norm_w = (const uint16_t *)norm_w_dev, c.eps = eps, c.partial = (float *)(mem + o_part), c.ss = (float *)(mem + o_ss);
        c.seg_mode = seg_mode, c.seg_end0 = seg_end0, c.seg_end1 = seg_end1, c.mode = mode;
        c.base = (const uint16_t *)base_or_residual_dev, c.dst = (uint16_t *)out_dev;
        rc = lora_apply(c, (hipStream_t)stream);
    }
    const hipError_t se = hipStreamSynchronize((hipStream_t)stream);
    if (rc == TL_OK && se != hipSuccess) rc = fail(TL_ERR_HIP, std::string("lora_rows: ") + hipGetErrorString(se));
    return rc;
}

static int engine_paged_attention(tl_engine *e, int l, const uint16_t *q_t, const int32_t *block_row, const int32_t *ctx_dev, uint16_t *attn_t,
                                  int n, int ctx_hint) {
    const tl_engine_config &c = e->cfg;
    const int D = c.head_dim, Hq = c.num_heads, Hkv = c.num_kv_heads;
    if (e->kv_format == TL_KV_FP8_E4M3)
        return tl_paged_attention_fp8(q_t, e->layer_k(l), e->layer_ks(l), e->layer_v(l), e->layer_vs(l), block_row, ctx_dev, attn_t, Hq, n, D,
                                      c.num_pages, c.page_size, c.max_pages_per_seq, Hq, Hkv, 1.0f / sqrtf((float)D), 1, ctx_hint, e->attn_ws,
                                      e->attn_ws_bytes, e->stream);
    return tl_paged_attention(q_t, e->layer_k(l), e->layer_v(l), block_row, ctx_dev, attn_t, Hq, n, D, c.num_pages, c.page_size,
                              c.max_pages_per_seq, Hq, Hkv, 1.0f / sqrtf((float)D), 1, ctx_hint, TL_BF16, e->attn_ws, e->attn_ws_bytes, e->stream);
}
static void launch_qkv_post(tl_engine *e, int l, QkvPostArgs &q, int n) {
    q.key_scales = e->layer_ks(l);
    q.value_scales = e->layer_vs(l);
    switch (e->cfg.head_dim) {
        case 128:
            if (e->kv_format == TL_KV_FP8_E4M3) hipLaunchKernelGGL((qkv_post_kernel<8, true>), dim3(n), dim3(256), 0, e->stream, q);
            else hipLaunchKernelGGL((qkv_post_kernel<8>), dim3(n), dim3(256), 0, e->stream, q);
            break;
        case 64: hipLaunchKernelGGL((qkv_post_kernel<4>), dim3(n), dim3(256), 0, e->stream, q); break;
        default: hipLaunchKernelGGL((qkv_post_kernel<2>), dim3(n), dim3(256), 0, e->stream, q); break;
    }
}

struct PrefillSeq {
    int slot, start, row0, len;
};

static int lm_head_rows(tl_engine *e, const uint16_t *x, int rows) {
    Proj p = proj(e->head(), x, e->logits, rows);
    p.pro = PRO_RMSNORM, p.norm_w = e->final_norm;
    return engine_qmv(e->lin, p);
}

static int prefill_pass(tl_engine *e, const PrefillSeq *seqs, int n_seqs, const int32_t *tokens, int total, bool packed) {
    const tl_engine_config &c = e->cfg;
    SlotEdits ed;
    Pokes pk;
    for (int i = 0; i < n_seqs; ++i) {
        TL_TRY(table_rc(e->table.reserve(seqs[i].slot, seqs[i].start + seqs[i].len, ed)));
        pk.emplace_back(e->scratch_ctx + i, seqs[i].start + seqs[i].len);
    }
    TL_TRY(apply_edits(e, ed, pk));
    TL_TRY(poke(e, pk));
    TL_HIP(hipMemcpyAsync(e->prefill_tokens, tokens, (size_t)total * 4, hipMemcpyHostToDevice, e->stream));
    for (int i = 0; i < n_seqs; ++i) {
        if (!step_processes_slot(e, seqs[i].slot)) continue;
        const LogitMarkArgs mk{e->prefill_tokens + seqs[i].row0, seqs[i].len, c.vocab_size, e->sdev<uint32_t>(SB_PROCESS, e->settings.at.pen_history), (long)seqs[i].slot * c.vocab_size};
        hipLaunchKernelGGL(logit_mark_prompt_kernel, dim3(ceil_div(seqs[i].len, 256)), dim3(256), 0, e->stream, mk);
        TL_CHECK_LAUNCH("engine prompt marking");
    }

    const int D = c.head_dim, Hq = c.num_heads, Hkv = c.num_kv_heads;
    TL_TRY(tl_quantized_embedding(e->prefill_tokens, 0, e->embed.scales_dev, e->embed.biases_dev, e->embed.weight_dev, e->x,
                                  total, c.hidden_size, c.vocab_size, 128, 4, TL_BF16, e->stream));
    for (int i = 0; i < n_seqs; ++i)
        TL_REQUIRE(tl_paged_attention_workspace_bytes(Hq, seqs[i].len, D, c.page_size, c.max_pages_per_seq, Hq, Hkv, seqs[i].start + seqs[i].len) <=
                       e->attn_ws_bytes, std::string(packed ? "engine_prefill_packed" : "engine_prefill") + ": attention workspace too small");
    int lora_tiles = 0;
    std::vector<LoraTile> lora_list;
    {
        int row0[16], len[16], ad[16];
        bool any = false;
        for (int i = 0; i < n_seqs; ++i) {
            row0[i] = seqs[i].row0, len[i] = seqs[i].len, ad[i] = e->settings.slots[seqs[i].slot].lora;
            if (ad[i] >= 0) any = true, e->lora_prefill_rows += seqs[i].len;
        }
        if (any) {
            TL_REQUIRE(lora_build_tiles(n_seqs, row0, len, ad, lora_list) && (int)lora_list.size() <= lora_tiles_cap(e), "engine: bad LoRA tile list");
            lora_tiles = (int)lora_list.size();
            TL_HIP(hipMemcpyAsync(e->lora_tiles_prefill, lora_list.data(), lora_list.size() * sizeof(LoraTile), hipMemcpyHostToDevice, e->stream));
        }
    }
    const auto lora_on = [&](int l, int g) {
        if (lora_tiles == 0) return false;
        for (int i = 0; i < n_seqs; ++i) {
            const int a = e->settings.slots[seqs[i].slot].lora;
            if (a >= 0 && e->lora_ad[a].has[(size_t)l * tl_engine::LORA_GROUPS + g]) return true;
        }
        return false;
    };
    bool x_normed = false;
    for (int l = 0; l < c.num_layers; ++l) {
        const tl_layer_weights &w = e->layers[l];
        if (!x_normed) TL_TRY(tl_rms_norm(e->x, w.input_norm_dev, e->xn, total, c.hidden_size, c.rms_norm_eps, TL_BF16, e->stream));
        x_normed = false;
        TL_TRY(engine_gemm(e->lin, proj(w.wqkv, e->xn, e->qkv, total)));
        if (lora_on(l, tl_engine::LORA_QKV))
            TL_TRY(lora_group(e, l, tl_engine::LORA_QKV, e->lora_tiles_prefill, lora_tiles, total, e->xn, nullptr, TL_LORA_ADD, nullptr, e->qkv));
        for (int i = 0; i < n_seqs; ++i) {
            const int n = seqs[i].len, start = seqs[i].start;
            const int32_t *block_row = e->block_table + (size_t)seqs[i].slot * c.max_pages_per_seq;
            uint16_t *q_t = e->q_t + (size_t)seqs[i].row0 * Hq * D;
            uint16_t *attn_t = e->attn_t + (size_t)seqs[i].row0 * Hq * D;
            QkvPostArgs q{};
            q.qkv = e->qkv + (size_t)seqs[i].row0 * (Hq + 2 * Hkv) * D;
            q.q_norm_w = (const uint16_t *)w.q_norm_dev;
            q.k_norm_w = (const uint16_t *)w.k_norm_dev;
            q.q_t = q_t;
            q.key_pages = e->layer_k(l);
            q.value_pages = e->layer_v(l);
            q.block_row = block_row;
            q.T = n;
            q.start = start;
            q.page_size = c.page_size;
            q.max_pages = c.max_pages_per_seq;
            q.num_heads = Hq;
            q.num_kv_heads = Hkv;
            q.eps = c.rms_norm_eps;
            q.rope_base = c.rope_theta;
            launch_qkv_post(e, l, q, n);
            TL_CHECK_LAUNCH("engine qkv_post");
            TL_TRY(engine_paged_attention(e, l, q_t, block_row, e->scratch_ctx + i, attn_t, n, start + n));
            const long items = (long)Hq * n * (D / 8);
            hipLaunchKernelGGL(heads_to_rows_kernel, dim3(ceil_div(items, 256)), dim3(256), 0, e->stream, attn_t,
                               e->attn + (size_t)seqs[i].row0 * Hq * D, Hq, n, D);
        }
        bool h_normed = false;
        Proj po = proj(w.wo, e->attn, e->h, total);
        po.epi = EPI_RESIDUAL, po.residual = e->x, po.norm_out = w.post_norm_dev, po.out_w = e->xn;
        if (lora_on(l, tl_engine::LORA_O)) {
            TL_TRY(lora_group(e, l, tl_engine::LORA_O, e->lora_tiles_prefill, lora_tiles, total, e->attn, nullptr, TL_LORA_RESIDUAL_PRE, e->x, e->lora_tmp));
            po.residual = e->lora_tmp;
        }
        TL_TRY(engine_gemm(e->lin, po, &h_normed));
        if (!h_normed) TL_TRY(tl_rms_norm(e->h, w.post_norm_dev, e->xn, total, c.hidden_size, c.rms_norm_eps, TL_BF16, e->stream));
        if (e->is_moe(l)) {
            TL_TRY(engine_moe_mlp(e, l, e->xn, e->h, e->x, total, nullptr));
        } else {
            TL_REQUIRE(w.wgu.weight_dev != nullptr, "engine: a layer has neither a dense MLP nor experts (tl_engine_set_moe_layer)");
            Proj pg = proj(w.wgu, e->xn, e->act, total);
            pg.epi = EPI_SWIGLU;
            if (lora_on(l, tl_engine::LORA_GU)) {
                pg.out = e->lin.gu, pg.epi = EPI_STORE;
                TL_TRY(engine_gemm(e->lin, pg));
                TL_TRY(lora_group(e, l, tl_engine::LORA_GU, e->lora_tiles_prefill, lora_tiles, total, e->xn, nullptr, TL_LORA_SWIGLU, e->lin.gu, e->act));
            } else {
                TL_TRY(engine_gemm(e->lin, pg));
            }
            Proj pd = proj(w.wdown, e->act, e->x, total);
            pd.epi = EPI_RESIDUAL, pd.residual = e->h, pd.norm_out = l + 1 < c.num_layers ? e->layers[l + 1].input_norm_dev : nullptr, pd.out_w = e->xn;
            if (lora_on(l, tl_engine::LORA_DOWN)) {
                TL_TRY(lora_group(e, l, tl_engine::LORA_DOWN, e->lora_tiles_prefill, lora_tiles, total, e->act, nullptr, TL_LORA_RESIDUAL_PRE, e->h, e->lora_tmp));
                pd.residual = e->lora_tmp;
            }
            TL_TRY(engine_gemm(e->lin, pd, &x_normed));
        }
        TL_CHECK_LAUNCH(packed ? "engine packed prefill layer" : "engine prefill layer");
    }
    for (int i = 0; i < n_seqs; ++i) {
        e->table.appended(seqs[i].slot, tokens + seqs[i].row0, seqs[i].len, !e->lora_slot(seqs[i].slot));
        e->settings.appended(seqs[i].slot, true);
        pk.emplace_back(e->context_lens + seqs[i].slot, seqs[i].start + seqs[i].len);
    }
    TL_TRY(poke(e, pk));
    e->stats.prefill_tokens += total;
    return TL_OK;
}

static int prefill_first_token(tl_engine *e, int slot, int row, const char *what) {
    launch_logit_chain(e, e->logits + (size_t)row * e->cfg.vocab_size, row, 1, slot, 0, e->h, nullptr, 0, nullptr, nullptr, step_features(e, slot, 1), nullptr);
    TL_CHECK_LAUNCH(what);
    e->table.slots[slot].produced += 1;
    e->settings.pending_produced(slot);
    return TL_OK;
}

static int prefill_impl(tl_engine *e, int slot, const int32_t *tokens, int n, int logits_mode) {
    TL_TRY(slot_check_feeds(e, slot));
// ... 944 lines not shown
```

tiny-llm_amd/csrc/engine_kernels.h:

```cpp
#pragma once
#include <type_traits>
#include "common.h"
#include "kv8.h"

namespace tl {

constexpr float ENG_LOG2E = 1.44269504089f;
constexpr int AD_RQ = 4;

template <int VD>
__device__ __forceinline__ void load_row(const uint16_t *src, float (&f)[VD]) {
    uint16_t raw[VD];
    if constexpr (VD == 8) {
        *reinterpret_cast<uint4 *>(raw) = *reinterpret_cast<const uint4 *>(src);
    } else if constexpr (VD == 4) {
        *reinterpret_cast<uint2 *>(raw) = *reinterpret_cast<const uint2 *>(src);
    } else if constexpr (VD == 2) {
        *reinterpret_cast<uint32_t *>(raw) = *reinterpret_cast<const uint32_t *>(src);
    } else {
#pragma unroll
        for (int i = 0; i < VD; ++i) raw[i] = src[i];
    }
#pragma unroll
    for (int i = 0; i < VD; ++i) f[i] = BF16::to_float(raw[i]);
}

template <int VD>
__device__ __forceinline__ void store_row(uint16_t *dst, const float (&f)[VD]) {
    uint16_t raw[VD];
#pragma unroll
    for (int i = 0; i < VD; ++i) raw[i] = BF16::from_float(f[i]);
    if constexpr (VD == 8) {
        *reinterpret_cast<uint4 *>(dst) = *reinterpret_cast<const uint4 *>(raw);
    } else if constexpr (VD == 4) {
        *reinterpret_cast<uint2 *>(dst) = *reinterpret_cast<const uint2 *>(raw);
    } else if constexpr (VD == 2) {
        *reinterpret_cast<uint32_t *>(dst) = *reinterpret_cast<const uint32_t *>(raw);
    } else {
#pragma unroll
        for (int i = 0; i < VD; ++i) dst[i] = raw[i];
    }
}

template <int VD>
__device__ __forceinline__ void rope_factors(int t, int pos, float base, float (&cs)[VD], float (&sn)[VD]) {
    constexpr int half = 8 * VD;
    const float lb = log2f(base);
#pragma unroll
    for (int i = 0; i < VD; ++i) {
        const int item = (t & 7) * VD + i;
        const float fp = -(float)item / (float)half;
        const float angle = (float)pos * exp2f(fp * lb);
        sincosf(angle, &sn[i], &cs[i]);
    }
}

template <int VD>
__device__ __forceinline__ void head_norm_rope(const uint16_t *src, const uint16_t *w, int t, float eps,
                                               const float (&cs)[VD], const float (&sn)[VD], float (&out)[VD]) {
    constexpr int D = 16 * VD;
    float f[VD], g[VD];
    load_row<VD>(src + t * VD, f);
    load_row<VD>(w + t * VD, g);
    float ss = 0.f;
#pragma unroll
    for (int i = 0; i < VD; ++i) ss += f[i] * f[i];
    ss = group16_sum(ss);
    const float inv = rsqrtf(ss / (float)D + eps);
#pragma unroll
    for (int i = 0; i < VD; ++i) {
        const float n = bf16_round(f[i] * inv * g[i]);
        const float partner = dpp_row_ror<8>(n);
        const float r = (t < 8) ? (n * cs[i] - partner * sn[i]) : (n * cs[i] + partner * sn[i]);
        out[i] = bf16_round(r);
    }
}

static __global__ __launch_bounds__(256) void rope_table_kernel(float2 *__restrict__ table, int max_pos, int half, float base) {
    const long idx = (long)blockIdx.x * 256 + threadIdx.x;
    if (idx >= (long)max_pos * half) return;
    const int pos = (int)(idx / half);
    const int item = (int)(idx - (long)pos * half);
    const float fp = -(float)item / (float)half;
    const float angle = (float)pos * exp2f(fp * log2f(base));
    float s, c;
    sincosf(angle, &s, &c);
    table[idx] = make_float2(c, s);
}

template <int VD>
__device__ __forceinline__ void rope_from_table(const float2 *__restrict__ row, int t, float (&cs)[VD], float (&sn)[VD]) {
    const float2 *p = row + (t & 7) * VD;
#pragma unroll
    for (int i = 0; i < VD; ++i) {
        const float2 v = p[i];
        cs[i] = v.x;
        sn[i] = v.y;
    }
}

template <int N>
__device__ __forceinline__ float row_ror(float v) {
    return __builtin_bit_cast(float, __builtin_amdgcn_update_dpp(0, __builtin_bit_cast(int, v), 0x120 + N, 0xf, 0xf, false));
}
__device__ __forceinline__ float group16_allsum(float v) {
    v += row_ror<8>(v);
    v += row_ror<4>(v);
    v += row_ror<2>(v);
    v += row_ror<1>(v);
    return v;
}

constexpr int ATTN_WS_PAD = 4;
struct AttnDecodeArgs {
    const uint16_t *qkv;
    const uint16_t *q_norm_w, *k_norm_w;
    uint16_t *key_pages, *value_pages;
    const int32_t *block_table;
    const int32_t *context_lens;
    uint16_t *out;
    float *ws;
    const float2 *rope_cur;
    int page_size, max_pages, num_heads, num_kv_heads;
    float scale, eps, rope_base;
    int n_splits, n_row_chunks, tokens_per_split;
    int split_shift;
    int rep;
    int page_shift;
// ... 582 lines not shown
            if (((cur ^ old) >> (16 * h)) & 0xffffu) {
                if (written[2 * i + h]) ++doubles, at = 2 * i + h;
                else written[2 * i + h] = 1, ++fresh;
            }
        }
        shadow[i] = cur;
    }
    if (fresh) atomicAdd(&report[3], fresh);
    if (doubles) {
        atomicAdd(&report[0], doubles);
        const unsigned long long before = atomicMin(&report[1], (unsigned long long)launch_idx);
        if ((unsigned long long)launch_idx <= before) report[2] = (unsigned long long)region_id, report[4] = at;
    }
}

static __global__ __launch_bounds__(1024) void prof_reduce_kernel(prof_t *buf, int n_wg, prof_t *out_pair) {
    __shared__ prof_t s_min[16], s_max[16];
    prof_t lo = ~0ull, hi = 0ull;
    for (int i = threadIdx.x; i < n_wg; i += 1024) {
        lo = min(lo, buf[2 * i]);
        hi = max(hi, buf[2 * i + 1]);
        buf[2 * i] = 0;
        buf[2 * i + 1] = 0;
    }
#pragma unroll
    for (int o = 32; o > 0; o >>= 1) {
        lo = min(lo, (prof_t)__shfl_xor((unsigned long long)lo, o, 64));
        hi = max(hi, (prof_t)__shfl_xor((unsigned long long)hi, o, 64));
    }
    if ((threadIdx.x & 63) == 0) {
        s_min[threadIdx.x >> 6] = lo;
        s_max[threadIdx.x >> 6] = hi;
    }
    __syncthreads();
    if (threadIdx.x == 0) {
        for (int w = 1; w < 16; ++w) {
            lo = min(lo, s_min[w]);
            hi = max(hi, s_max[w]);
        }
        out_pair[0] = lo;
        out_pair[1] = hi;
    }
}

struct QkvPostArgs {
    const uint16_t *qkv;
    const uint16_t *q_norm_w, *k_norm_w;
    uint16_t *q_t;
    uint16_t *key_pages, *value_pages;
    const int32_t *block_row;
    int T, start, page_size, max_pages, num_heads, num_kv_heads;
    float eps, rope_base;
    float *key_scales, *value_scales;
};

template <int VD, bool KV8 = false>
static __global__ __launch_bounds__(256) void qkv_post_kernel(const QkvPostArgs p) {
    static_assert(!KV8 || VD == 8, "FP8 pages: head dimension 128");
    constexpr int D = 16 * VD;
    const int r = blockIdx.x;
    const int g = threadIdx.x >> 4;
    const int t = threadIdx.x & 15;
    const int Hq = p.num_heads, Hkv = p.num_kv_heads;
    const int pos = p.start + r;
    const uint16_t *row = p.qkv + (long)r * (Hq + 2 * Hkv) * D;
    float cs[VD], sn[VD];
    rope_factors<VD>(t, pos, p.rope_base, cs, sn);
    const int lp = pos / p.page_size;
    const int slot = pos - lp * p.page_size;
    const int page_id = lp < p.max_pages ? p.block_row[lp] : -1;
    for (int h = g; h < Hq + 2 * Hkv; h += 16) {
        float v[VD];
        if (h < Hq) {
            head_norm_rope<VD>(row + (long)h * D, p.q_norm_w, t, p.eps, cs, sn, v);
            store_row<VD>(p.q_t + ((long)h * p.T + r) * D + t * VD, v);
        } else if (h < Hq + Hkv) {
            head_norm_rope<VD>(row + (long)h * D, p.k_norm_w, t, p.eps, cs, sn, v);
            const long prow = ((long)max(page_id, 0) * Hkv + (h - Hq)) * p.page_size + slot;
            if constexpr (KV8) {
                u32x2 codes;
                float sc, deq[8];
                kv8_quantize_row16(v, codes, sc, deq);
                if (page_id >= 0) {
                    *reinterpret_cast<u32x2 *>(reinterpret_cast<uint8_t *>(p.key_pages) + prow * D + t * VD) = codes;
                    if (t == 0) p.key_scales[prow] = sc;
                }
            } else if (page_id >= 0)
                store_row<VD>(p.key_pages + prow * D + t * VD, v);
        } else {
            load_row<VD>(row + (long)h * D + t * VD, v);
            const long prow = ((long)max(page_id, 0) * Hkv + (h - Hq - Hkv)) * p.page_size + slot;
            if constexpr (KV8) {
                u32x2 codes;
                float sc, deq[8];
                kv8_quantize_row16(v, codes, sc, deq);
                if (page_id >= 0) {
                    *reinterpret_cast<u32x2 *>(reinterpret_cast<uint8_t *>(p.value_pages) + prow * D + t * VD) = codes;
                    if (t == 0) p.value_scales[prow] = sc;
                }
            } else if (page_id >= 0)
                store_row<VD>(p.value_pages + prow * D + t * VD, v);
        }
    }
}

static __global__ __launch_bounds__(256) void heads_to_rows_kernel(const uint16_t *__restrict__ in, uint16_t *__restrict__ out,
                                                            int H, int T, int D) {
    const int vpr = D / 8;
    const long total = (long)H * T * vpr;
    const long idx = (long)blockIdx.x * 256 + threadIdx.x;
    if (idx >= total) return;
    const int v = (int)(idx % vpr);
    const int h = (int)((idx / vpr) % H);
    const int t = (int)(idx / ((long)vpr * H));
    *reinterpret_cast<uint4 *>(out + ((long)t * H + h) * D + v * 8) =
        *reinterpret_cast<const uint4 *>(in + ((long)h * T + t) * D + v * 8);
}

static __global__ __launch_bounds__(256) void residual_add_kernel(const uint16_t *__restrict__ a, const uint16_t *__restrict__ b,
                                                           uint16_t *__restrict__ out, long n8) {
    const long idx = (long)blockIdx.x * 256 + threadIdx.x;
    if (idx >= n8) return;
    uint16_t x[8], y[8], o[8];
    *reinterpret_cast<uint4 *>(x) = reinterpret_cast<const uint4 *>(a)[idx];
    *reinterpret_cast<uint4 *>(y) = reinterpret_cast<const uint4 *>(b)[idx];
#pragma unroll
    for (int e = 0; e < 8; ++e) o[e] = BF16::from_float(BF16::to_float(x[e]) + BF16::to_float(y[e]));
    reinterpret_cast<uint4 *>(out)[idx] = *reinterpret_cast<const uint4 *>(o);
}

static __global__ __launch_bounds__(256) void weight_rows_kernel(const uint16_t *__restrict__ x, const uint16_t *__restrict__ w,
                                                          uint16_t *__restrict__ out, long n8, int chunks_per_row, int frag) {
    const long idx = (long)blockIdx.x * 256 + threadIdx.x;
    if (idx >= n8) return;
    uint16_t a[8], g[8], o[8];
    *reinterpret_cast<uint4 *>(a) = reinterpret_cast<const uint4 *>(x)[idx];
    const int row = (int)(idx / chunks_per_row), ch = (int)(idx - (long)row * chunks_per_row);
    if (w) {
        *reinterpret_cast<uint4 *>(g) = reinterpret_cast<const uint4 *>(w)[ch];
#pragma unroll
        for (int e = 0; e < 8; ++e) o[e] = BF16::from_float(BF16::to_float(a[e]) * BF16::to_float(g[e]));
    } else {
#pragma unroll
// ... 185 lines not shown
```

tiny-llm_amd/csrc/qmm.hip:

```cpp
#include "common.h"
#include "qmv.h"

namespace tl {

template <typename TT>
__global__ __launch_bounds__(256) void qmm_vanilla_kernel(const uint16_t *__restrict__ scales,
                                                          const uint16_t *__restrict__ biases,
                                                          const uint16_t *__restrict__ a,
                                                          const uint32_t *__restrict__ b, uint16_t *__restrict__ out,
                                                          int M, int N, int K) {
    const int k = blockIdx.x * 64 + (threadIdx.x & 63);
    const int i = blockIdx.y * 4 + (threadIdx.x >> 6);
    if (i >= M || k >= K) return;
    const int G = N / 128;
    const uint32_t *bw = b + (size_t)k * (N / 8);
    const uint16_t *ar = a + (size_t)i * N;
    float sum = 0.f;
    for (int g = 0; g < G; ++g) {
        const float scale = TT::to_float(scales[(size_t)k * G + g]);
        const float bias = TT::to_float(biases[(size_t)k * G + g]);
        for (int w = 0; w < 16; ++w) {
            const uint32_t packed = bw[g * 16 + w];
            const uint4 av = *reinterpret_cast<const uint4 *>(ar + g * 128 + w * 8);
            const uint32_t aw[4] = {av.x, av.y, av.z, av.w};
// ... 434 lines not shown
    return TL_OK;
}

int qmm_bf16_epilogue(const void *scales, const void *biases, const uint16_t *A, const uint32_t *b, uint16_t *O, int M, int N, int K,
                      int epi, const uint16_t *residual, void *workspace, size_t workspace_bytes, hipStream_t st, const uint16_t *norm_w,
                      uint16_t *norm_out, float norm_eps, bool *norm_done) {
    if (norm_done) *norm_done = false;
    if (M <= 8 || epi == EPI_STORE) return fail(TL_ERR_INVALID, "qmm_bf16_epilogue: for more than 8 rows and a real epilogue");
    if (epi == EPI_RESIDUAL && !residual) return fail(TL_ERR_INVALID, "qmm_bf16_epilogue: residual rows missing");
    if (epi == EPI_SWIGLU && (K % 2) != 0) return fail(TL_ERR_INVALID, "qmm_bf16_epilogue: SwiGLU needs an even number of weight rows");
    auto S = (const uint16_t *)scales;
    auto Bi = (const uint16_t *)biases;
    const int mt = mfma_mt(M);
    const int nw = mfma_nw(M, K);
    const int split = split_k_policy(M, N, K);
    const dim3 grid(ceil_div(K, 32 * nw), ceil_div(M, 32 * mt), split), block(64 * nw);
    const int psize = N / split;
    const size_t pstride = (size_t)M * K;
    if (split > 1) {
        const size_t need = (size_t)split * M * K * 2;
        if (!workspace || workspace_bytes < need) return fail(TL_ERR_INVALID, "qmm_bf16_epilogue: split-K workspace is missing or too small");
        uint16_t *dst = (uint16_t *)workspace;
        if (nw == 8) hipLaunchKernelGGL((qmm_mfma_kernel<BF16, 4, 8>), grid, block, 0, st, S, Bi, A, b, dst, M, N, K, psize, pstride, nullptr, qmm_xcd_remap());
        else if (mt == 1) hipLaunchKernelGGL((qmm_mfma_kernel<BF16, 1>), grid, block, 0, st, S, Bi, A, b, dst, M, N, K, psize, pstride, nullptr, qmm_xcd_remap());
        else if (mt == 2) hipLaunchKernelGGL((qmm_mfma_kernel<BF16, 2>), grid, block, 0, st, S, Bi, A, b, dst, M, N, K, psize, pstride, nullptr, qmm_xcd_remap());
        else hipLaunchKernelGGL((qmm_mfma_kernel<BF16, 4>), grid, block, 0, st, S, Bi, A, b, dst, M, N, K, psize, pstride, nullptr, qmm_xcd_remap());
        const size_t elements = (size_t)M * K;
        if (elements % 8 != 0 || (((uintptr_t)O | (uintptr_t)dst | (uintptr_t)residual) & 15) != 0)
            return fail(TL_ERR_INVALID, "qmm_bf16_epilogue: rows x features must be a multiple of 8 and the rows 16-byte aligned");
        const dim3 rg(ceil_div(elements / 8, 256));
        if (epi == EPI_RESIDUAL && norm_w && norm_out && norm_done && K % 8 == 0 && K > 2048 && K <= 4096 && (((uintptr_t)norm_w | (uintptr_t)norm_out) & 15) == 0) {
            hipLaunchKernelGGL((splitk_reduce_residual_norm_kernel<BF16>), dim3(M), dim3((K / 8 + 63) / 64 * 64), 0, st, dst, O, elements, split, residual, norm_w, norm_out, K, norm_eps);
            *norm_done = true;
            return TL_OK;
        }
        if (epi == EPI_SWIGLU) hipLaunchKernelGGL((splitk_reduce_epi_kernel<BF16, EPI_SWIGLU>), rg, dim3(256), 0, st, dst, O, elements, split, residual);
        else hipLaunchKernelGGL((splitk_reduce_epi_kernel<BF16, EPI_RESIDUAL>), rg, dim3(256), 0, st, dst, O, elements, split, residual);
        return TL_OK;
    }
#define QMM_EPI_LAUNCH(EPIv)                                                                                                     \
    if (nw == 8) hipLaunchKernelGGL((qmm_mfma_kernel<BF16, 4, 8, EPIv>), grid, block, 0, st, S, Bi, A, b, O, M, N, K, psize, pstride, residual, qmm_xcd_remap()); \
    else if (mt == 1) hipLaunchKernelGGL((qmm_mfma_kernel<BF16, 1, 4, EPIv>), grid, block, 0, st, S, Bi, A, b, O, M, N, K, psize, pstride, residual, qmm_xcd_remap()); \
    else if (mt == 2) hipLaunchKernelGGL((qmm_mfma_kernel<BF16, 2, 4, EPIv>), grid, block, 0, st, S, Bi, A, b, O, M, N, K, psize, pstride, residual, qmm_xcd_remap()); \
    else hipLaunchKernelGGL((qmm_mfma_kernel<BF16, 4, 4, EPIv>), grid, block, 0, st, S, Bi, A, b, O, M, N, K, psize, pstride, residual, qmm_xcd_remap());
    if (epi == EPI_SWIGLU) {
        QMM_EPI_LAUNCH(EPI_SWIGLU)
    } else {
        QMM_EPI_LAUNCH(EPI_RESIDUAL)
    }
#undef QMM_EPI_LAUNCH
    return TL_OK;
}

template <typename TT>
static int run_gather_qmv(const void *scales, const void *biases, const void *a, const uint32_t *b, const int32_t *expert_ids,
                          void *out, int M, int N, int K, int num_experts, hipStream_t st, int a_rows_div = 1) {
    QmvArgs args{};
    args.scales = (const uint16_t *)scales;
    args.biases = (const uint16_t *)biases;
    args.a = (const uint16_t *)a;
    args.b = b;
    args.out = (uint16_t *)out;
    args.M = 1;
    args.N = N;
    args.K = K;
    args.expert_ids = expert_ids;
    args.num_experts = num_experts;
    args.a_rows_div = a_rows_div;
    const QmvPlan pl = qmv_plan(1, N, K);
    if (pl.lds > 150 * 1024) return fail(TL_ERR_UNSUPPORTED, "gather_quantized_matvec: reduction dimension too large");
    const dim3 grid(pl.blocks, M), block(256);
#define GQ_CASE(WNv, RPLv)                                                                                          \
    if (pl.WN == WNv && pl.RPL == RPLv) {                                                                           \
        auto kern = qmv_kernel<TT, 1, WNv, RPLv, PRO_NONE, EPI_STORE>;                                              \
        if (pl.lds > 64 * 1024)                                                                                     \
            (void)hipFuncSetAttribute((const void *)kern, hipFuncAttributeMaxDynamicSharedMemorySize, (int)pl.lds); \
        hipLaunchKernelGGL(kern, grid, block, pl.lds, st, args);                                                    \
        return TL_OK;                                                                                               \
    }
    GQ_CASE(1, 2) GQ_CASE(1, 1) GQ_CASE(2, 1) GQ_CASE(4, 1)
#undef GQ_CASE
    return fail(TL_ERR_UNSUPPORTED, "gather_quantized_matvec: no GEMV configuration for this shape");
}

int gather_qmv_bf16(const void *scales, const void *biases, const uint16_t *a, const uint32_t *b, const int32_t *expert_ids,
                    uint16_t *out, int M, int N, int K, int num_experts, int a_rows_div, hipStream_t st) {
    if (M > 65535) return fail(TL_ERR_INVALID, "grouped-expert matvec: at most 65535 rows per launch");
    if (M == 0 || K == 0) return TL_OK;
    return run_gather_qmv<BF16>(scales, biases, a, b, expert_ids, out, M, N, K, num_experts, st, a_rows_div);
}

}

using namespace tl;

extern "C" int tl_gather_quantized_matvec(const void *scales, const void *biases, const void *a, const uint32_t *b,
                                          const int32_t *expert_ids, void *out, int M, int N, int K, int num_experts,
                                          int group_size, int bits, tl_dtype dtype, void *stream) {
    TL_REQUIRE(dtype == TL_F16 || dtype == TL_BF16, "gather_quantized_matvec: scales must be float16 or bfloat16");
    TL_REQUIRE(bits == 4, "gather_quantized_matvec: bits must be 4");
    TL_REQUIRE(group_size == 128, "gather_quantized_matvec: group_size must be 128");
    TL_REQUIRE(scales && biases && a && b && expert_ids && out, "gather_quantized_matvec: null pointer");
    TL_REQUIRE(M >= 0 && K >= 0 && N > 0 && num_experts > 0, "gather_quantized_matvec: bad shape");
    TL_REQUIRE(N % 128 == 0, "gather_quantized_matvec: N must be divisible by group_size");
    TL_REQUIRE(M <= 65535, "gather_quantized_matvec: at most 65535 rows per call");
    if (M == 0 || K == 0) return TL_OK;
// ... 44 lines not shown
```

tiny-llm_amd/csrc/qmv.h:

```cpp
#pragma once
#include "common.h"

namespace tl {

enum { PRO_NONE = 0, PRO_RMSNORM = 1, PRO_ATTN_MERGE = 2, PRO_RMS_WEIGHTED = 3 };
enum { EPI_STORE = 0, EPI_RESIDUAL = 1, EPI_SWIGLU = 2 };

struct QmvArgs {
    const uint16_t *scales;
    const uint16_t *biases;
    const uint16_t *a;
    const uint32_t *b;
    uint16_t *out;
    const uint16_t *norm_w;
    const uint16_t *residual;
    float eps;
    int M, N, K;
    prof_t *prof;
    prof_t *trace;
    const int32_t *expert_ids;
    int num_experts;
    int a_rows_div;
};

// ... 290 lines not shown
                    const float r = TT::to_float(TT::from_float(v));
                    p.out[o] = TT::from_float(TT::to_float(p.residual[o]) + r);
                }
            } else {
                if (cl == 0 && row_ok[rp] && m < p.M) p.out[(size_t)m * K + row[rp]] = TT::from_float(v);
            }
        }
    }
    prof_end(p.prof, prof_t0);
}

struct QmvPlan {
    int MR, WN, RPL, RB, blocks;
    size_t lds;
};
inline QmvPlan qmv_plan(int M, int N, int K) {
    QmvPlan pl;
    pl.MR = M <= 1 ? 1 : (M <= 2 ? 2 : (M <= 4 ? 4 : 8));
    const int J = (N + 511) / 512;
    int rb = 4;
    const int cands[3] = {32, 16, 8};
    for (int c : cands) {
        if ((K + c - 1) / c >= 768) {
            rb = c;
            break;
        }
    }
    if (rb == 32) {
        pl.WN = 1; pl.RPL = 2;
    } else if (rb == 16) {
        pl.WN = 1; pl.RPL = 1;
    } else if (rb == 8) {
        pl.WN = 2; pl.RPL = 1;
    } else {
        pl.WN = 4; pl.RPL = 1;
    }
    if (pl.WN > J) {
        pl.WN = J >= 2 ? 2 : 1;
        pl.RPL = 1;
    }
    pl.RB = 4 * (4 / pl.WN) * pl.RPL;
    pl.blocks = (K + pl.RB - 1) / pl.RB;
    pl.lds = qmv_lds_bytes(pl.MR, N, pl.WN, pl.RPL);
    return pl;
}

int launch_qmv_fused_bf16(const QmvArgs &args, int pro, int epi, hipStream_t st);

int gather_qmv_bf16(const void *scales, const void *biases, const uint16_t *a, const uint32_t *b, const int32_t *expert_ids,
                    uint16_t *out, int M, int N, int K, int num_experts, int a_rows_div, hipStream_t st);
int qmm_bf16_epilogue(const void *scales, const void *biases, const uint16_t *a, const uint32_t *b, uint16_t *out, int M, int N, int K,
                      int epi, const uint16_t *residual, void *workspace, size_t workspace_bytes, hipStream_t st, const uint16_t *norm_w = nullptr,
                      uint16_t *norm_out = nullptr, float norm_eps = 0.f, bool *norm_done = nullptr);
}
```

tiny-llm_amd/extensions_hip/tiny_llm_ext_hip/__init__.py:

```python

from __future__ import annotations

import ctypes
import os
from pathlib import Path

import torch

_LIB_NAME = "libtinyllm_hip.so"
_LIB_PATH = Path(__file__).resolve().parent / _LIB_NAME

if not _LIB_PATH.exists():
    raise ImportError(
        f"{_LIB_PATH} is missing: build it with `python -c 'import __graft_entry__ as g; g.build()'` "
        "or `make -C tiny-llm_amd/csrc` (hipcc, gfx950). There is no CPU fallback."
    )

_lib = ctypes.CDLL(str(_LIB_PATH), mode=os.RTLD_LOCAL if hasattr(os, "RTLD_LOCAL") else 0)

_c_void_p = ctypes.c_void_p
_c_int = ctypes.c_int
_c_float = ctypes.c_float
_c_size_t = ctypes.c_size_t

TL_F32, TL_F16, TL_BF16 = 0, 1, 2
_DTYPES = {torch.float32: TL_F32, torch.float16: TL_F16, torch.bfloat16: TL_BF16}

_SIGNATURES = {
    "tl_last_error": (ctypes.c_char_p, []),
    "tl_abi_version": (_c_int, []),
    "tl_load_library": (_c_int, [ctypes.c_char_p]),
    "tl_quantized_matmul": (
        _c_int,
        [_c_void_p] * 5 + [_c_int] * 5 + [_c_int, _c_int, _c_int, _c_void_p, _c_size_t, _c_void_p],
    ),
    "tl_quantized_matmul_workspace_bytes": (_c_size_t, [_c_int] * 6),
    "tl_gather_quantized_matvec": (_c_int, [_c_void_p] * 6 + [_c_int] * 7 + [_c_void_p]),
    "tl_quantized_matmul_split_k": (_c_int, [_c_int] * 5),
    "tl_quantized_embedding": (_c_int, [_c_void_p, _c_int] + [_c_void_p] * 4 + [_c_int] * 6 + [_c_void_p]),
    "tl_rms_norm": (_c_int, [_c_void_p] * 3 + [_c_int, _c_int, _c_float, _c_int, _c_void_p]),
    "tl_rope": (_c_int, [_c_void_p] * 3 + [_c_int] * 5 + [_c_float, _c_int, _c_int, _c_void_p]),
    "tl_swiglu": (_c_int, [_c_void_p] * 3 + [_c_size_t, _c_int, _c_void_p]),
    "tl_decode_attention": (_c_int, [_c_void_p] * 5 + [_c_int] * 6 + [_c_float, _c_int, _c_int, _c_int, _c_void_p]),
    "tl_paged_cache_update": (_c_int, [_c_void_p] * 2 + [_c_int] * 8 + [_c_void_p]),
    "tl_paged_attention": (
        _c_int,
        [_c_void_p] * 6 + [_c_int] * 8 + [_c_float, _c_int, _c_int, _c_int, _c_void_p, _c_size_t, _c_void_p],
    ),
    "tl_paged_attention_workspace_bytes": (_c_size_t, [_c_int] * 8),
    "tl_paged_attention_waves": (_c_int, [_c_int]),
    "tl_kv_fp8_quantize_rows": (_c_int, [_c_void_p, _c_void_p, _c_void_p, ctypes.c_long, _c_int, _c_void_p]),
    "tl_kv_fp8_dequantize_rows": (_c_int, [_c_void_p, _c_void_p, _c_void_p, ctypes.c_long, _c_int, _c_void_p]),
    "tl_paged_cache_update_fp8": (_c_int, [_c_void_p] * 3 + [_c_int] * 7 + [_c_void_p]),
    "tl_paged_attention_fp8": (
        _c_int,
        [_c_void_p] * 8 + [_c_int] * 8 + [_c_float, _c_int, _c_int, _c_void_p, _c_size_t, _c_void_p],
    ),
}



class TlW4(ctypes.Structure):
    _fields_ = [("weight_dev", _c_void_p), ("scales_dev", _c_void_p), ("biases_dev", _c_void_p),
                ("rows", _c_int), ("cols", _c_int)]


class TlLayerWeights(ctypes.Structure):
    _fields_ = [("wqkv", TlW4), ("wo", TlW4), ("wgu", TlW4), ("wdown", TlW4),
                ("input_norm_dev", _c_void_p), ("post_norm_dev", _c_void_p),
                ("q_norm_dev", _c_void_p), ("k_norm_dev", _c_void_p)]


class TlMoeWeights(ctypes.Structure):
    _fields_ = [("router", TlW4), ("gate_dev", _c_void_p), ("up_dev", _c_void_p), ("down_dev", _c_void_p),
                ("gate_scales_dev", _c_void_p), ("gate_biases_dev", _c_void_p), ("up_scales_dev", _c_void_p),
                ("up_biases_dev", _c_void_p), ("down_scales_dev", _c_void_p), ("down_biases_dev", _c_void_p),
                ("num_experts", _c_int), ("experts_per_token", _c_int), ("intermediate_size", _c_int),
                ("norm_topk_prob", _c_int)]


class TlEngineConfig(ctypes.Structure):
    _fields_ = [("hidden_size", _c_int), ("num_layers", _c_int), ("num_heads", _c_int), ("num_kv_heads", _c_int),
                ("head_dim", _c_int), ("intermediate_size", _c_int), ("vocab_size", _c_int),
                ("rope_theta", _c_float), ("rms_norm_eps", _c_float),
                ("page_size", _c_int), ("num_pages", _c_int), ("max_batch", _c_int), ("max_pages_per_seq", _c_int),
                ("max_prefill_rows", _c_int)]


class TlEngineStats(ctypes.Structure):
    _fields_ = [("pages_in_use", _c_int), ("pages_free", _c_int), ("peak_pages_in_use", _c_int),
                ("page_allocations", ctypes.c_long), ("reused_page_allocations", ctypes.c_long),
                ("decode_steps", ctypes.c_long), ("graph_captures", ctypes.c_long), ("graph_replays", ctypes.c_long),
                ("prefill_tokens", ctypes.c_long), ("kv_bytes", _c_size_t), ("workspace_bytes", _c_size_t),
                ("graph_cache_flushes", ctypes.c_long), ("aql_steps", ctypes.c_long)]


class TlStepProfile(ctypes.Structure):
    _fields_ = [("kernel_us", ctypes.c_double * 8), ("launches", _c_int * 8), ("gemv_bytes", ctypes.c_double * 5),
                ("span_us", ctypes.c_double), ("clock_khz", _c_int), ("n_splits", _c_int)]


class TlStepCheck(ctypes.Structure):
    _fields_ = [("launches", _c_int), ("written_once_plan", _c_int), ("n_splits", _c_int), ("double_writes", ctypes.c_long),
                ("elements_written", ctypes.c_long), ("first_launch", _c_int), ("first_kind", _c_int), ("first_region", _c_int),
                ("first_offset", ctypes.c_long)]


TL_MAX_TOP_LOGPROBS = 20
TL_MAX_LOGIT_BIAS = 1024
# ... 57 lines not shown

TL_MAX_STOP_IDS = 16
TL_MAX_STOP_STRINGS = 16
TL_MAX_STOP_BYTES = 1024
STOP_REASONS = ("none", "id", "string", "length")


class TlStopState(ctypes.Structure):
    _fields_ = [("reason", ctypes.c_int32), ("index", ctypes.c_int32), ("generated", ctypes.c_int32), ("context", ctypes.c_int32),
                ("text_bytes", ctypes.c_uint32), ("cut_bytes", ctypes.c_uint32)]


class TlAttentionInfo(ctypes.Structure):
    _fields_ = [("n_splits", _c_int), ("tokens_per_split", _c_int), ("heads_per_workgroup", _c_int),
                ("launches", _c_int)]


class TlVerifyResult(ctypes.Structure):
    _fields_ = [("count", ctypes.c_int32), ("ids", ctypes.c_int32 * 8)]


_P = ctypes.POINTER
_SIGNATURES.update({
    "tl_tiled_w4_create": (_c_int, [_P(TlW4), _c_void_p, _P(_c_void_p)]),
    "tl_tiled_w4_destroy": (None, [_c_void_p]),
    "tl_decode_linear_workspace_bytes": (_c_size_t, [_c_int, _c_int, _c_int]),
    "tl_decode_linear": (_c_int, [_c_void_p, _c_void_p, _c_void_p, _c_int, _c_int, _c_int, _c_void_p, _c_void_p, _c_float,
                                  _c_int, _c_void_p, _c_size_t, _c_void_p, _P(TlLinearInfo)]),
    "tl_decode_linear_ex": (_c_int, [_c_void_p, _c_void_p, _c_void_p, _c_int, _c_int, _c_int, _c_void_p, _c_void_p, _c_float,
                                     _c_int, _c_void_p, _c_size_t, _c_void_p, _P(TlLinearEx), _P(TlLinearInfo)]),
    "tl_prefill_weights_bf16": (_c_int, [_P(TlW4), _c_void_p, _c_void_p]),
    "tl_prefill_matmul_bf16": (_c_int, [_c_void_p, _c_void_p, _c_void_p, _c_int, _c_int, _c_int, _c_int, _c_void_p, _c_void_p]),
    "tl_decode_gemv_variant_compiled": (_c_int, [_c_int, _c_int, _c_int, _c_int]),
    "tl_decode_attention_fused_workspace_bytes": (_c_size_t, [_c_int, _c_int, _c_int]),
    "tl_decode_attention_fused": (_c_int, [_c_void_p] * 8 + [_c_int] * 6 + [_c_float, _c_float, _c_int, _c_void_p, _c_size_t,
                                                             _c_void_p, _P(TlAttentionInfo)]),
    "tl_engine_profile_step": (_c_int, [_c_void_p, _c_int, _P(TlStepProfile)]),
    "tl_engine_check_step": (_c_int, [_c_void_p, _c_int, _P(TlStepCheck)]),
    "tl_engine_create": (_c_int, [_P(TlEngineConfig), _P(TlLayerWeights), _P(TlW4), _c_void_p, _P(TlW4), _c_void_p,
                                  _P(_c_void_p)]),
    "tl_engine_create_kv": (_c_int, [_P(TlEngineConfig), _P(TlLayerWeights), _P(TlW4), _c_void_p, _P(TlW4), _c_void_p, _c_int,
                                     _P(_c_void_p)]),
    "tl_engine_kv_format": (_c_int, [_c_void_p]),
    "tl_decode_attention_fused_fp8": (_c_int, [_c_void_p] * 10 + [_c_int] * 6 + [_c_float, _c_float, _c_int, _c_void_p, _c_size_t,
                                                                  _c_void_p, _P(TlAttentionInfo)]),
    "tl_engine_set_moe_layer": (_c_int, [_c_void_p, _c_int, _P(TlMoeWeights)]),
    "tl_decode_gemv_plan": (_c_int, [_c_int, _c_int, _c_int, _P(_c_int)]),
    "tl_decode_batched_plan": (_c_int, [_c_int, _c_int, _c_int, _P(_c_int)]),
    "tl_decode_batched_variant_compiled": (_c_int, [_c_int, _c_int]),
    "tl_decode_streaming_plan": (_c_int, [_c_int, _c_int, _c_int, _P(_c_int)]),
    "tl_decode_streaming_variant_compiled": (_c_int, [_c_int, _c_int]),
    "tl_decode_attention_plan": (_c_int, [_c_int, _c_int, _c_int, _c_int, _P(_c_int)]),
    "tl_engine_set_option": (_c_int, [_c_void_p, ctypes.c_char_p, _c_int]),
    "tl_engine_destroy": (None, [_c_void_p]),
    "tl_engine_synchronize": (_c_int, [_c_void_p]),
    "tl_engine_begin": (_c_int, [_c_void_p, _c_int]),
    "tl_engine_reserve": (_c_int, [_c_void_p, _c_int, _c_int]),
    "tl_engine_release": (_c_int, [_c_void_p, _c_int]),
    "tl_engine_rewind": (_c_int, [_c_void_p, _c_int, _c_int]),
    "tl_engine_context_len": (_c_int, [_c_void_p, _c_int]),
    "tl_engine_move": (_c_int, [_c_void_p, _c_int, _c_int]),
    "tl_engine_fork": (_c_int, [_c_void_p, _c_int, _c_int]),
    "tl_engine_read_pending": (_c_int, [_c_void_p, _c_int, _P(ctypes.c_int32)]),
    "tl_engine_prefix_cache": (_c_int, [_c_void_p, _c_int, _c_int]),
    "tl_engine_prefix_attach": (_c_int, [_c_void_p, _c_int, _P(ctypes.c_int32), _c_int, _P(_c_int)]),
    "tl_engine_prefix_extend": (_c_int, [_c_void_p, _c_int, _P(ctypes.c_int32), _c_int]),
    "tl_engine_prefix_clear": (_c_int, [_c_void_p]),
    "tl_engine_prefix_stats": (_c_int, [_c_void_p, _P(TlPrefixStats)]),
    "tl_kv_copy_rows": (_c_int, [_c_void_p, _c_int, _c_int, _c_int, _c_int, _c_int, _c_int, _c_void_p]),
    "tl_engine_swap_space": (_c_int, [_c_void_p, _c_int]),
    "tl_engine_park": (_c_int, [_c_void_p, _c_int]),
    "tl_engine_unpark": (_c_int, [_c_void_p, _c_int]),
    "tl_engine_slot_parked": (_c_int, [_c_void_p, _c_int]),
    "tl_engine_step_pages": (_c_int, [_c_void_p, _c_int, _P(_c_int), _P(_c_int)]),
    "tl_engine_swap_stats": (_c_int, [_c_void_p, _P(TlSwapStats)]),
    "tl_kv_page_record_bytes": (_c_size_t, [_c_void_p, _c_int, _c_int, _c_int]),
    "tl_kv_gather_pages": (_c_int, [_c_void_p, _c_void_p, _c_int, _c_int, _c_int, _c_void_p, _c_int, _c_int, _c_void_p, _c_size_t, _c_void_p]),
    "tl_kv_scatter_pages": (_c_int, [_c_void_p, _c_void_p, _c_int, _c_int, _c_int, _c_void_p, _c_int, _c_int, _c_void_p, _c_size_t, _c_void_p]),
    "tl_engine_prefill": (_c_int, [_c_void_p, _c_int, _P(ctypes.c_int32), _c_int, _c_int]),
    "tl_engine_prefill_packed": (_c_int, [_c_void_p, _c_int, _P(ctypes.c_int), _P(ctypes.c_int32), _P(ctypes.c_int), _P(ctypes.c_int)]),
    "tl_engine_verify": (_c_int, [_c_void_p, _c_int, _P(ctypes.c_int32), _c_int, _P(ctypes.c_int32)]),
    "tl_engine_verify_sampled": (_c_int, [_c_void_p, _c_int, _P(ctypes.c_int32), _c_int, _c_void_p, ctypes.c_float, _c_int, ctypes.c_float,
                                          _P(ctypes.c_int32), _P(_c_int)]),
    "tl_engine_verify_batch": (_c_int, [_c_void_p, _c_int, _P(ctypes.c_int), _P(ctypes.c_int32), _P(ctypes.c_int), _c_int, _P(TlVerifyResult)]),
    "tl_verify_attention_rows": (_c_int, [_c_void_p] * 8 + [_c_int, _P(ctypes.c_int), _P(ctypes.c_int), _P(ctypes.c_int), _c_void_p] + [_c_int] * 4 +
                                 [_c_float, _c_float, _c_void_p, _P(TlAttentionInfo)]),
    "tl_verify_accept_rows": (_c_int, [_c_void_p, _c_int, _c_int, _P(ctypes.c_int), _P(ctypes.c_int), _c_void_p, _c_void_p, _c_void_p]),
    "tl_engine_set_token": (_c_int, [_c_void_p, _c_int, ctypes.c_int32]),
    "tl_engine_set_sampling": (_c_int, [_c_void_p, _c_int, _c_float, _c_int, _c_float, ctypes.c_uint64]),
    "tl_sample_logits": (_c_int, [_c_void_p, _c_int, _c_int] + [_c_void_p] * 7),
    "tl_engine_set_logprobs": (_c_int, [_c_void_p, _c_int, _c_int]),
    "tl_engine_set_penalties": (_c_int, [_c_void_p, _c_int, _c_float, _c_float, _c_float]),
    "tl_engine_set_logit_bias": (_c_int, [_c_void_p, _c_int, _P(ctypes.c_int32), _P(_c_float), _c_int]),
    "tl_process_logits": (_c_int, [_c_void_p, _c_int, _c_int] + [_c_void_p] * 9),
    "tl_engine_set_truncation": (_c_int, [_c_void_p, _c_int, _c_float, _c_float]),
    "tl_engine_set_mirostat": (_c_int, [_c_void_p, _c_int, _c_float, _c_float]),
    "tl_engine_mirostat_mu": (_c_int, [_c_void_p, _c_int, _P(_c_float)]),
    "tl_engine_copy_filtered_logits": (_c_int, [_c_void_p, _c_void_p, _c_int]),
    "tl_truncate_rows": (_c_int, [_c_void_p, _c_int, _c_int] + [_c_void_p] * 7),
    "tl_spec_sample_rows": (_c_int, [_c_void_p, _c_void_p, _c_int, _c_int] + [_c_void_p] * 12),
    "tl_mirostat_update_rows": (_c_int, [_c_void_p, _c_int, _c_int] + [_c_void_p] * 7),
    "tl_vocab_create": (_c_int, [_c_int, _c_void_p, _c_void_p, _c_void_p, _P(_c_void_p)]),
    "tl_vocab_destroy": (None, [_c_void_p]),
    "tl_grammar_create": (_c_int, [_c_void_p, _c_int, _c_void_p, _c_void_p, _c_int, _c_void_p, _c_int, _c_void_p, _P(_c_void_p)]),
    "tl_grammar_destroy": (None, [_c_void_p]),
    "tl_engine_set_grammar": (_c_int, [_c_void_p, _c_int, _c_void_p]),
# ... 696 lines not shown
    if num_heads % num_kv_heads != 0 or query.shape[0] % num_heads != 0 or key_pages.shape[1] != num_kv_heads:
        raise RuntimeError("paged_attention_fp8: incompatible head counts")
    if query.shape[2] != 128 or key_pages.shape[3] != 128:
        raise RuntimeError("paged_attention_fp8: FP8 pages need head dimension 128")
    if query.shape[0] // num_heads != block_table.shape[0] or block_table.shape[0] != context_lens.shape[0]:
        raise RuntimeError("paged_attention_fp8: q batch size must match block_table and context_lens")
    tensors = (query, key_pages, key_scales, value_pages, value_scales, block_table, context_lens)
    _require_gpu("paged_attention_fp8", *tensors)
    if not all(t.is_contiguous() for t in tensors):
        raise RuntimeError("paged_attention_fp8: every tensor must be contiguous")
    N, L, D = query.shape
    P, _, page_size, _ = key_pages.shape
    max_pages = block_table.shape[1]
    out = torch.empty_like(query)
    ws_bytes = _lib.tl_paged_attention_workspace_bytes(N, L, D, page_size, max_pages, num_heads, num_kv_heads, int(max_context_hint))
    ws = _workspace(ws_bytes, query.device)
    _check(_lib.tl_paged_attention_fp8(
        _ptr(query), _ptr(key_pages), _ptr(key_scales), _ptr(value_pages), _ptr(value_scales), _ptr(block_table), _ptr(context_lens),
        _ptr(out), N, L, D, P, page_size, max_pages, int(num_heads), int(num_kv_heads), float(scale), int(bool(is_causal)),
        int(max_context_hint), _ptr(ws) if ws is not None else None, ws.numel() if ws is not None else 0, _stream()))
    return out


def decode_attention_fused_fp8(qkv: torch.Tensor, q_norm: torch.Tensor, k_norm: torch.Tensor, key_pages: torch.Tensor,
                               key_scales: torch.Tensor, value_pages: torch.Tensor, value_scales: torch.Tensor,
                               block_table: torch.Tensor, context_lens: torch.Tensor, *, num_heads: int, num_kv_heads: int,
                               rope_theta: float, eps: float, max_context: int) -> tuple[torch.Tensor, dict]:
    _require_gpu("decode_attention_fused_fp8", qkv, q_norm, k_norm, key_pages, key_scales, value_pages, value_scales, block_table, context_lens)
    B = int(qkv.shape[0])
    P, Hkv, page, D = (int(x) for x in key_pages.shape)
    if D != 128 or Hkv != num_kv_heads or tuple(value_pages.shape) != tuple(key_pages.shape) \
            or tuple(key_scales.shape) != (P, Hkv, page) or tuple(value_scales.shape) != (P, Hkv, page):
        raise RuntimeError("decode_attention_fused_fp8: pages [P, num_kv_heads, page_size, 128] uint8 and scales [P, num_kv_heads, page_size]")
    if qkv.dim() != 2 or qkv.shape[1] != (num_heads + 2 * num_kv_heads) * D:
        raise RuntimeError("decode_attention_fused_fp8: qkv must be [batch, (Hq + 2 Hkv) * D]")
    for name, t, dt in (("qkv", qkv, torch.bfloat16), ("q_norm", q_norm, torch.bfloat16), ("k_norm", k_norm, torch.bfloat16),
                        ("key_pages", key_pages, torch.uint8), ("value_pages", value_pages, torch.uint8),
                        ("key_scales", key_scales, torch.float32), ("value_scales", value_scales, torch.float32)):
        if t.dtype != dt or not t.is_contiguous():
            raise RuntimeError(f"decode_attention_fused_fp8: {name} must be contiguous {dt}")
    if block_table.dtype != torch.int32 or context_lens.dtype != torch.int32 or block_table.dim() != 2 \
            or block_table.shape[0] != B or tuple(context_lens.shape) != (B,):
        raise RuntimeError("decode_attention_fused_fp8: block_table [B, max_pages] and context_lens [B] must be int32")
    out = torch.empty((B, num_heads * D), dtype=torch.bfloat16, device=qkv.device)
    ws = _workspace(_lib.tl_decode_attention_fused_workspace_bytes(B, num_heads, D), qkv.device)
    info = TlAttentionInfo()
    _check(_lib.tl_decode_attention_fused_fp8(_ptr(qkv), _ptr(q_norm), _ptr(k_norm), _ptr(key_pages), _ptr(key_scales), _ptr(value_pages),
                                              _ptr(value_scales), _ptr(block_table.contiguous()), _ptr(context_lens), _ptr(out), B,
                                              num_heads, num_kv_heads, D, page, int(block_table.shape[1]), float(rope_theta), float(eps),
                                              int(max_context), _ptr(ws), ws.numel(), _stream(), ctypes.byref(info)))
    return out, {name: getattr(info, name) for name, _ in info._fields_}


def paged_attention_waves(waves: int = 0) -> int:
    return int(_lib.tl_paged_attention_waves(int(waves)))


def sample_logits(logits: torch.Tensor, temperature, top_k, top_p, seed, position) -> torch.Tensor:
    if logits.dtype != torch.bfloat16 or logits.dim() != 2 or not logits.is_cuda:
        raise ValueError("sample_logits takes a [rows, vocab] bf16 tensor on the GPU")
    logits = logits.contiguous()
    rows, dev = logits.shape[0], logits.device

    def per_row(v, dtype):
        t = torch.as_tensor(v, dtype=dtype).reshape(-1)
        if t.numel() == 1:
            t = t.expand(rows)
        if t.numel() != rows:
            raise ValueError("a sampling parameter needs one value per row")
        return t.contiguous().to(dev)

    seeds = [int(s) & 0xFFFFFFFFFFFFFFFF for s in (seed if hasattr(seed, "__len__") else [seed] * rows)]
    seed_t = torch.tensor([s - (1 << 64) if s >= 1 << 63 else s for s in seeds], dtype=torch.int64).to(dev)
    if seed_t.numel() != rows:
        raise ValueError("a sampling parameter needs one value per row")
    t_t, k_t, p_t, pos_t = per_row(temperature, torch.float32), per_row(top_k, torch.int32), per_row(top_p, torch.float32), per_row(position, torch.int32)
    ids = torch.empty(rows, dtype=torch.int32, device=dev)
    check(_lib.tl_sample_logits(logits.data_ptr(), rows, logits.shape[1], t_t.data_ptr(), k_t.data_ptr(), p_t.data_ptr(), seed_t.data_ptr(),
                                pos_t.data_ptr(), ids.data_ptr(), _stream()))
    return ids


def spec_sample_rows(target: torch.Tensor, draft: torch.Tensor, proposal, temperature, top_k, top_p, draft_temperature, draft_top_k,
                     draft_top_p, seed, position):
    for t in (target, draft):
        if t.dtype != torch.bfloat16 or t.dim() != 2 or not t.is_cuda:
            raise ValueError("spec_sample_rows takes [rows, vocab] bf16 tensors on the GPU")
    if target.shape != draft.shape or target.device != draft.device:
        raise ValueError("spec_sample_rows: target and draft rows must have one shape and one device")
    target, draft = target.contiguous(), draft.contiguous()
    rows, dev = target.shape[0], target.device

    def per_row(v, dtype):
        t = torch.as_tensor(v, dtype=dtype).reshape(-1)
        if t.numel() == 1:
            t = t.expand(rows)
        if t.numel() != rows:
            raise ValueError("a speculative-sampling parameter needs one value per row")
        return t.contiguous().to(dev)

    seeds = [int(s) & 0xFFFFFFFFFFFFFFFF for s in (seed if hasattr(seed, "__len__") else [seed] * rows)]
    if len(seeds) != rows:
        raise ValueError("a speculative-sampling parameter needs one value per row")
    seed_t = torch.tensor([s - (1 << 64) if s >= 1 << 63 else s for s in seeds], dtype=torch.int64).to(dev)
    x_t, pos_t = per_row(proposal, torch.int32), per_row(position, torch.int32)
    tt, tk, tp = per_row(temperature, torch.float32), per_row(top_k, torch.int32), per_row(top_p, torch.float32)
# ... 243 lines not shown
```

tiny-llm_amd/tiny_llm_hip/engine.py:

```python

from __future__ import annotations

import ctypes
import math
import os
from typing import Any, NamedTuple, Sequence

import torch

from . import scheduler
from .scheduler import RequestSettings
from ._ext import tiny_llm_ext_hip as _ext

_lib = _ext.lib()


def _w4(weight: torch.Tensor, scales: torch.Tensor, biases: torch.Tensor) -> "_ext.TlW4":
    rows, words = weight.shape
    return _ext.TlW4(weight.data_ptr(), scales.data_ptr(), biases.data_ptr(), rows, words * 8)


def _bits(t: torch.Tensor) -> torch.Tensor:
    return t.view(torch.int32) if t.dtype != torch.int32 else t

# ... 513 lines not shown
    def logits(self, rows: int = 1) -> torch.Tensor:
        out = torch.empty((rows, self.vocab_size), dtype=torch.bfloat16, device=self.device)
        torch.cuda.current_stream().synchronize()
        _ext.check(_lib.tl_engine_copy_logits(self._h, out.data_ptr(), rows))
        self.synchronize()
        return out

    def logits_buffer(self, rows: int) -> torch.Tensor:
        out = torch.empty((rows, self.vocab_size), dtype=torch.bfloat16, device=self.device)
        torch.cuda.current_stream().synchronize()
        return out

    def copy_logits_into(self, dst: torch.Tensor, rows: int = 1) -> None:
        if dst.dtype != torch.bfloat16 or not dst.is_cuda or not dst.is_contiguous() or dst.numel() < rows * self.vocab_size:
            raise ValueError(f"copy_logits_into needs a contiguous bf16 tensor of at least {rows} x {self.vocab_size} elements on the GPU")
        _ext.check(_lib.tl_engine_copy_logits(self._h, dst.data_ptr(), rows))

    def processed_logits(self, rows: int = 1) -> torch.Tensor:
        out = torch.empty((rows, self.vocab_size), dtype=torch.bfloat16, device=self.device)
        torch.cuda.current_stream().synchronize()
        _ext.check(_lib.tl_engine_copy_processed_logits(self._h, out.data_ptr(), rows))
        self.synchronize()
        return out

    def filtered_logits(self, rows: int = 1) -> torch.Tensor:
        out = torch.empty((rows, self.vocab_size), dtype=torch.bfloat16, device=self.device)
        torch.cuda.current_stream().synchronize()
        _ext.check(_lib.tl_engine_copy_filtered_logits(self._h, out.data_ptr(), rows))
        self.synchronize()
        return out

    def synchronize(self) -> None:
        _ext.check(_lib.tl_engine_synchronize(self._h))

    def step_bytes(self, batch: int | None = None) -> int:
        return int(_lib.tl_engine_step_bytes(self._h, batch or self.max_batch))

    PROFILE_KINDS = ("gemv_qkv", "gemv_o", "gemv_gate_up", "gemv_down", "gemv_lm_head", "attention",
                     "attention_merge", "step_end")

    def profile_step(self, batch: int | None = None) -> dict:
        p = _ext.TlStepProfile()
        _ext.check(_lib.tl_engine_profile_step(self._h, batch or self.max_batch, ctypes.byref(p)))
        out = {"span_us": p.span_us, "clock_khz": p.clock_khz, "n_splits": p.n_splits, "kinds": {}}
        for i, name in enumerate(self.PROFILE_KINDS):
            out["kinds"][name] = {"us": p.kernel_us[i], "launches": p.launches[i],
                                  "bytes": p.gemv_bytes[i] if i < 5 else 0.0}
        return out

    def check_step(self, batch: int | None = None) -> dict:
        c = _ext.TlStepCheck()
        _ext.check(_lib.tl_engine_check_step(self._h, batch or self.max_batch, ctypes.byref(c)))
        return {name: getattr(c, name) for name, _ in c._fields_}

    def replay_route(self) -> str:
        return (_lib.tl_engine_replay_route(self._h) or b"").decode()

    def stats(self) -> dict:
        s = _ext.TlEngineStats()
        _ext.check(_lib.tl_engine_get_stats(self._h, ctypes.byref(s)))
        return {name: getattr(s, name) for name, _ in s._fields_}

    def generate(self, prompt: Sequence[int], max_new_tokens: int, *, slot: int = 0, chunk: int | None = None,
                 temperature: float = 0.0, top_k: int | None = None, top_p: float | None = None, seed: int = 0,
                 logprobs: int | None = None, repetition_penalty: float = 1.0, presence_penalty: float = 0.0,
                 frequency_penalty: float = 0.0, logit_bias=None, grammar: "Grammar | None" = None, min_p: float = 0.0,
                 typical_p: float = 1.0, mirostat_tau: float = 0.0, mirostat_eta: float = 0.1, lora: int | None = None,
                 stop: "StopSet | None" = None, decode_block: int = 32):
        if stop is not None and (isinstance(decode_block, bool) or not isinstance(decode_block, int) or decode_block < 1):
            raise ValueError("generate: decode_block is a positive int")
        settings = request_settings(
            {"temperature": temperature, "top_k": top_k, "top_p": top_p, "seed": seed, "min_p": min_p, "typical_p": typical_p,
             "mirostat_tau": mirostat_tau, "mirostat_eta": mirostat_eta, "repetition_penalty": repetition_penalty,
             "presence_penalty": presence_penalty, "frequency_penalty": frequency_penalty, "logit_bias": logit_bias, "grammar": grammar,
             "lora": lora}, 1, vocab_size=self.vocab_size, logprobs=logprobs, stop=stop, limits=[max_new_tokens])[0]
        top_n = settings.top_n
        self.begin(slot)
        try:
            settings.apply(self, slot)
            prompt = [int(t) for t in prompt]
            matched = self.prefix_attach(slot, prompt) if self.prefix_cache_enabled and prompt else 0
            self.prefill(slot, prompt[matched:], chunk=chunk)
            if stop is not None:
                left = max_new_tokens - 1
                state = self.stop_state(slot)
                while not state.stopped and left > 0:
                    steps = min(decode_block, left)
                    self.decode(steps, batch=slot + 1)
                    left -= steps
                    state = self.stop_state(slot)
                ids = self.read_tokens(slot, state.generated)
                self.last_stop_state = state
                if self.prefix_cache_enabled:
                    self.prefix_extend(slot, ids[:-1])
                return (ids, self.read_logprobs(slot, state.generated)) if top_n >= 0 else ids
            if max_new_tokens > 1:
                self.decode(max_new_tokens - 1, batch=slot + 1)
            ids = self.read_tokens(slot, max_new_tokens)
            if self.prefix_cache_enabled:
                self.prefix_extend(slot, ids[:-1])
            return (ids, self.read_logprobs(slot, max_new_tokens)) if top_n >= 0 else ids
        finally:
            self.release(slot)


class TokenLogprob(NamedTuple):
# ... 452 lines not shown
```

Baseline: 974.4 tokens/s.

## Fuse prefill QKV split-K reduce with norm/rope/KV write, attention writes rows directly

Prefill keeps the QKV GEMM split-K partials and reduces them inside a fused post-processing kernel that applies q/k norm, RoPE and the paged KV write. Paged attention gains output strides so results land directly in [token, heads*D] row layout, which removes a transpose before the O projection. Both paths sit behind new options that are on by default and only touch prefill. Decode-step throughput, which is the metric here, is essentially unaffected apart from the 128-token prefill share.

```diff
diff --git a/include/tinyllm_engine.h b/include/tinyllm_engine.h
--- a/include/tinyllm_engine.h
+++ b/include/tinyllm_engine.h
@@ -63,6 +63,8 @@
 int tl_engine_kv_format(const tl_engine *e);
 int tl_engine_set_moe_layer(tl_engine *e, int layer, const tl_moe_weights *w);
 int tl_engine_set_option(tl_engine *e, const char *name, int value);
+const char *tl_engine_option_names(void);
+const char *tl_engine_prefill_route(const tl_engine *e);
 void tl_engine_destroy(tl_engine *e);
 int tl_engine_synchronize(tl_engine *e);
 
@@ -326,6 +328,11 @@
                                   float eps, int max_context, void *workspace_dev, size_t workspace_bytes, void *stream,
                                   tl_attention_info *info);
 
+int tl_qkv_post_rows(const void *partials_dev, int slices, void *qkv_rows_dev, const void *q_norm_dev, const void *k_norm_dev, void *q_t_dev,
+                     void *key_pages_dev, float *key_scales_dev, void *value_pages_dev, float *value_scales_dev, const int32_t *block_row_dev,
+                     int T, int start, int page_size, int max_pages, int num_heads, int num_kv_heads, int head_dim, float rope_theta, float eps,
+                     int fused, void *stream);
+
 int tl_sample_logits(const void *logits_dev, int rows, int vocab, const float *temperature_dev, const int32_t *top_k_dev,
                      const float *top_p_dev, const uint64_t *seed_dev, const int32_t *position_dev, int32_t *ids_dev, void *stream);
 
diff --git a/include/tinyllm_hip.h b/include/tinyllm_hip.h
--- a/include/tinyllm_hip.h
+++ b/include/tinyllm_hip.h
@@ -73,6 +73,12 @@
                            int L, int D, int num_pages, int page_size, int max_pages, int num_heads, int num_kv_heads, float scale,
                            int is_causal, int max_context_hint, void *workspace, size_t workspace_bytes, void *stream);
 
+int tl_paged_attention_strided(const void *q, const void *key_pages, const float *key_scales, const void *value_pages,
+                               const float *value_scales, const int32_t *block_table, const int32_t *context_lens, void *out, int N,
+                               int L, int D, int num_pages, int page_size, int max_pages, int num_heads, int num_kv_heads, float scale,
+                               int is_causal, int max_context_hint, tl_dtype dtype, void *workspace, size_t workspace_bytes,
+                               long out_row_stride, long out_head_stride, void *stream);
+
 
 #ifdef __cplusplus
 }
diff --git a/tiny-llm_amd/csrc/attention.hip b/tiny-llm_amd/csrc/attention.hip
--- a/tiny-llm_amd/csrc/attention.hip
+++ b/tiny-llm_amd/csrc/attention.hip
@@ -150,7 +150,8 @@
     const typename TT::storage *__restrict__ value_pages, const int32_t *__restrict__ block_table,
     const int32_t *__restrict__ context_lens, typename TT::storage *__restrict__ out, float *__restrict__ ws, int L,
     int D, int page_size, int max_pages, int num_heads, int num_kv_heads, float scale, int is_causal, int n_splits,
-    int n_row_chunks, const float *__restrict__ key_scales = nullptr, const float *__restrict__ value_scales = nullptr) {
+    int n_row_chunks, const float *__restrict__ key_scales, const float *__restrict__ value_scales, long out_row_stride,
+    long out_head_stride) {
     static_assert(!KV8 || (VD == 8 && VEC), "FP8 pages: head dimension 128");
     using S = typename TT::storage;
     extern __shared__ __attribute__((aligned(16))) float psm[];
@@ -288,9 +289,10 @@
             gl += src[D + 1] * f;
             vs += src[d] * f;
         }
-        const long orow = ((long)b * num_heads + kvh * rep + hq_o) * L + qp_o;
+        const long n_o = (long)b * num_heads + kvh * rep + hq_o;
+        const long orow = n_o * L + qp_o;
         if (n_splits == 1) {
-            out[orow * D + d] = TT::from_float(gl == 0.f ? 0.f : vs / gl);
+            out[n_o * out_head_stride + qp_o * out_row_stride + d] = TT::from_float(gl == 0.f ? 0.f : vs / gl);
         } else {
             float *w = ws + (orow * n_splits + split) * stride;
             w[d] = vs;
@@ -305,8 +307,9 @@
 template <typename TT>
 __global__ __launch_bounds__(128) void paged_merge_kernel(const float *__restrict__ ws,
                                                           typename TT::storage *__restrict__ out, int D,
-                                                          int n_splits) {
+                                                          int n_splits, int L, long out_row_stride, long out_head_stride) {
     const long orow = blockIdx.x;
+    typename TT::storage *__restrict__ dst = out + (orow / L) * out_head_stride + (orow % L) * out_row_stride;
     const int stride = D + 2;
     const float *base = ws + orow * n_splits * stride;
     float gm = -1e30f;
@@ -318,7 +321,7 @@
             gl += base[s * stride + D + 1] * f;
             vs += base[s * stride + d] * f;
         }
-        out[orow * D + d] = TT::from_float(gl == 0.f ? 0.f : vs / gl);
+        dst[d] = TT::from_float(gl == 0.f ? 0.f : vs / gl);
     }
 }
 
@@ -338,8 +341,8 @@
     const uint16_t *__restrict__ q, const void *__restrict__ key_pages_v, const void *__restrict__ value_pages_v,
     const int32_t *__restrict__ block_table, const int32_t *__restrict__ context_lens, uint16_t *__restrict__ out,
     float *__restrict__ ws, int n_splits, int L, int page_size, int page_shift, int max_pages, int num_heads, int num_kv_heads,
-    float scale, int is_causal, int xcd_remap, const float *__restrict__ key_scales = nullptr,
-    const float *__restrict__ value_scales = nullptr) {
+    float scale, int is_causal, int xcd_remap, const float *__restrict__ key_scales, const float *__restrict__ value_scales,
+    long out_row_stride, long out_head_stride) {
     constexpr int D = 128;
     using KVE = typename std::conditional<KV8, uint8_t, uint16_t>::type;
     using KVC = typename std::conditional<KV8, u32x2, u32x4>::type;
@@ -728,7 +731,7 @@
             }
             continue;
         }
-        uint16_t *orow = out + ((long)n * L + qrow[rb]) * D;
+        uint16_t *orow = out + (long)n * out_head_stride + (long)qrow[rb] * out_row_stride;
         const float inv = run_sum[rb] == 0.f ? 0.f : 1.0f / run_sum[rb];
 #pragma unroll
         for (int db = 0; db < 4; ++db) {
@@ -850,8 +853,11 @@
                                 const float *value_scales, const int32_t *block_table, const int32_t *context_lens, void *out, int N,
                                 int L, int D, int num_pages, int page_size, int max_pages, int num_heads, int num_kv_heads, float scale,
                                 int is_causal, int max_context_hint, tl_dtype dtype, void *workspace, size_t workspace_bytes,
-                                void *stream) {
+                                void *stream, long out_row_stride = 0, long out_head_stride = 0) {
     const bool kv8 = key_scales != nullptr;
+    if (out_row_stride == 0 && out_head_stride == 0) out_row_stride = D, out_head_stride = (long)L * D;
+    TL_REQUIRE(out_row_stride >= D && out_head_stride >= D && out_row_stride % 8 == 0 && out_head_stride % 8 == 0,
+               "paged_attention: output strides are multiples of 8 elements, at least the head dimension");
     TL_REQUIRE(dtype == TL_F32 || dtype == TL_BF16,
                "paged_attention: q, key_pages, and value_pages must have the same float32 or bfloat16 dtype");
     TL_REQUIRE(q && key_pages && value_pages && block_table && context_lens && out, "paged_attention: null pointer");
@@ -887,7 +893,7 @@
         hipLaunchKernelGGL((paged_fa_bf16_d128_kernel<ONEP, QRv, K8>), grid, dim3(256), 0, st, (const uint16_t *)q, key_pages,  \
                            value_pages, block_table, context_lens, (uint16_t *)out, (float *)workspace, fa_splits, L, page_size, \
                            page_shift, max_pages, num_heads, num_kv_heads, scale, is_causal, fa_xcd_remap, key_scales,            \
-                           value_scales)
+                           value_scales, out_row_stride, out_head_stride)
 #define FA_LAUNCH8(K8)                                                                                                           \
         do {                                                                                                                         \
             static bool attr_set_dev[64] = {};        \
@@ -903,7 +909,7 @@
             hipLaunchKernelGGL((paged_fa_bf16_d128_kernel<true, 1, K8, 8>), grid, dim3(512), fa_pipe_lds_bytes(), st,                \
                                (const uint16_t *)q, key_pages, value_pages, block_table, context_lens, (uint16_t *)out,             \
                                (float *)workspace, fa_splits, L, page_size, page_shift, max_pages, num_heads, num_kv_heads, scale,   \
-                               is_causal, fa_xcd_remap, key_scales, value_scales);                                                   \
+                               is_causal, fa_xcd_remap, key_scales, value_scales, out_row_stride, out_head_stride);                  \
         } while (0)
         if (w8) {
             if (kv8) FA_LAUNCH8(true);
@@ -918,7 +924,7 @@
         TL_CHECK_LAUNCH("paged_attention(prefill)");
         if (fa_splits > 1) {
             hipLaunchKernelGGL((paged_merge_kernel<BF16>), dim3(N * L), dim3(128), 0, st, (const float *)workspace,
-                               (uint16_t *)out, D, fa_splits);
+                               (uint16_t *)out, D, fa_splits, L, out_row_stride, out_head_stride);
             TL_CHECK_LAUNCH("paged_attention(prefill merge)");
         }
         return TL_OK;
@@ -937,12 +943,13 @@
     hipLaunchKernelGGL((paged_decode_kernel<TT, VDv, VECv>), grid, block, lds, st, (const typename TT::storage *)q, \
                        (const typename TT::storage *)key_pages, (const typename TT::storage *)value_pages,         \
                        block_table, context_lens, (typename TT::storage *)out, ws, L, D, page_size, max_pages,     \
-                       num_heads, num_kv_heads, scale, is_causal, splits, row_chunks)
+                       num_heads, num_kv_heads, scale, is_causal, splits, row_chunks, nullptr, nullptr, out_row_stride,    \
+                       out_head_stride)
     if (kv8) {
         hipLaunchKernelGGL((paged_decode_kernel<BF16, 8, true, true>), grid, block, lds, st, (const uint16_t *)q,
                            (const uint16_t *)key_pages, (const uint16_t *)value_pages, block_table, context_lens, (uint16_t *)out, ws,
                            L, D, page_size, max_pages, num_heads, num_kv_heads, scale, is_causal, splits, row_chunks, key_scales,
-                           value_scales);
+                           value_scales, out_row_stride, out_head_stride);
     } else if (dtype == TL_BF16) {
         if (D == 128) PD_LAUNCH(BF16, 8, true);
         else if (D == 64) PD_LAUNCH(BF16, 4, true);
@@ -956,9 +963,10 @@
     TL_CHECK_LAUNCH("paged_attention(decode)");
     if (splits > 1) {
         if (dtype == TL_BF16) {
-            hipLaunchKernelGGL((paged_merge_kernel<BF16>), dim3(N * L), dim3(128), 0, st, ws, (uint16_t *)out, D, splits);
+            hipLaunchKernelGGL((paged_merge_kernel<BF16>), dim3(N * L), dim3(128), 0, st, ws, (uint16_t *)out, D, splits, L, out_row_stride,
+                               out_head_stride);
         } else {
-            hipLaunchKernelGGL((paged_merge_kernel<F32>), dim3(N * L), dim3(128), 0, st, ws, (float *)out, D, splits);
+            hipLaunchKernelGGL((paged_merge_kernel<F32>), dim3(N * L), dim3(128), 0, st, ws, (float *)out, D, splits, L, out_row_stride, out_head_stride);
         }
         TL_CHECK_LAUNCH("paged_attention(merge)");
     }
@@ -1023,3 +1031,16 @@
                                 page_size, max_pages, num_heads, num_kv_heads, scale, is_causal, max_context_hint, TL_BF16, workspace,
                                 workspace_bytes, stream);
 }
+
+extern "C" int tl_paged_attention_strided(const void *q, const void *key_pages, const float *key_scales, const void *value_pages,
+                                          const float *value_scales, const int32_t *block_table, const int32_t *context_lens, void *out,
+                                          int N, int L, int D, int num_pages, int page_size, int max_pages, int num_heads, int num_kv_heads,
+                                          float scale, int is_causal, int max_context_hint, tl_dtype dtype, void *workspace,
+                                          size_t workspace_bytes, long out_row_stride, long out_head_stride, void *stream) {
+    TL_REQUIRE((key_scales == nullptr) == (value_scales == nullptr), "paged_attention_strided: both scale arrays (FP8 pages) or neither");
+    TL_REQUIRE(!key_scales || (D == 128 && dtype == TL_BF16), "paged_attention_strided: FP8 pages need bfloat16 queries of head dimension 128");
+    TL_REQUIRE(out_row_stride > 0 && out_head_stride > 0, "paged_attention_strided: strides must be positive");
+    return paged_attention_impl(q, key_pages, value_pages, key_scales, value_scales, block_table, context_lens, out, N, L, D, num_pages,
+                                page_size, max_pages, num_heads, num_kv_heads, scale, is_causal, max_context_hint, dtype, workspace,
+                                workspace_bytes, stream, out_row_stride, out_head_stride);
+}
diff --git a/tiny-llm_amd/csrc/decode_linear.h b/tiny-llm_amd/csrc/decode_linear.h
--- a/tiny-llm_amd/csrc/decode_linear.h
+++ b/tiny-llm_amd/csrc/decode_linear.h
@@ -259,10 +259,16 @@
 
 constexpr int GEMM8_MIN_ROWS = 1792;
 static bool gemm8_wins(int M) { return M >= GEMM8_MIN_ROWS; }
-static int engine_gemm(LinearCtx &ctx, const Proj &p, bool *norm_done = nullptr) {
+struct GemmKept {
+    const uint16_t *partials = nullptr;
+    int slices = 0;
+    size_t plane = 0;
+};
+static int engine_gemm(LinearCtx &ctx, const Proj &p, bool *norm_done = nullptr, GemmKept *kept = nullptr) {
     const tl_w4 &w = *p.w;
     const int M = p.M;
     if (norm_done) *norm_done = false;
+    if (kept) *kept = GemmKept{};
     if (ctx.use_gemm8 && gemm8_wins(M)) {
         const auto wb = ctx.bf16w.find(w.weight_dev);
         if (wb != ctx.bf16w.end() && gemm8_applicable(M, w.rows, w.cols)) {
@@ -283,6 +289,18 @@
         return TL_OK;
     }
     uint16_t *plain = p.epi == EPI_STORE ? p.out : (p.epi == EPI_SWIGLU ? ctx.gu : ctx.tmp);
+    if (kept && p.epi == EPI_STORE && M > 8) {
+        int slices = 1;
+        size_t plane = 0;
+        TL_TRY(ensure_splitk(ctx, tl_quantized_matmul_workspace_bytes(M, w.cols, w.rows, TL_BF16, 1, 1)));
+        TL_TRY(qmm_bf16_keep_partials(w.scales_dev, w.biases_dev, p.a, w.weight_dev, M, w.cols, w.rows, ctx.splitk_ws, ctx.splitk_ws_bytes, ctx.stream,
+                                      &slices, &plane));
+        if (slices > 1) {
+            kept->partials = (const uint16_t *)ctx.splitk_ws, kept->slices = slices, kept->plane = plane;
+            TL_CHECK_LAUNCH("engine matmul");
+            return TL_OK;
+        }
+    }
     TL_TRY(engine_qmm(ctx, w, p.a, plain, M));
     if (p.epi == EPI_SWIGLU) {
         const long n4 = (long)M * (w.rows / 2) / 4;
diff --git a/tiny-llm_amd/csrc/engine.hip b/tiny-llm_amd/csrc/engine.hip
--- a/tiny-llm_amd/csrc/engine.hip
+++ b/tiny-llm_amd/csrc/engine.hip
@@ -124,6 +124,10 @@
     bool lm_tile_max_on = true;
     float *ss_x = nullptr, *ss_h = nullptr;
     bool attn_qkv_partials = true;
+    bool prefill_fa_rows = true, prefill_qkv_post_reduce = true;
+    struct PrefillRoute {
+        bool fa_rows = false, qkv_post_reduce = false;
+    } prefill_route;
     bool wo_merges_attn = true;
     int32_t *verify_ids = nullptr;
     struct SpecRecord {
@@ -1316,6 +1320,11 @@
     return TL_OK;
 }
 
+extern "C" const char *tl_engine_option_names() {
+    return "qmm3, qmm6, qmm7, gemm8, prefill_reduce_norm, prefill_fa_rows, prefill_qkv_post_reduce, attn_qkv_partials, lmhead_tile_max, "
+           "gemm_fused_epilogue, aql_fences";
+}
+
 extern "C" int tl_engine_set_option(tl_engine *e, const char *name, int value) {
     TL_REQUIRE(e && name, "engine_set_option: null argument");
     TL_REQUIRE(e->plans.empty() && e->stats.decode_steps == 0 && e->stats.prefill_tokens == 0,
@@ -1330,9 +1339,18 @@
     else if (n == "gemm_fused_epilogue") e->lin.gemm_fused_epilogue = on;
     else if (n == "gemm8") e->lin.use_gemm8 = on;
     else if (n == "prefill_reduce_norm") e->lin.fuse_reduce_norm = on;
+    else if (n == "prefill_fa_rows") e->prefill_fa_rows = on;
+    else if (n == "prefill_qkv_post_reduce") e->prefill_qkv_post_reduce = on;
     else if (n == "aql_fences") e->aql_fences.inner_acquire = e->aql_fences.inner_release = on ? HSA_FENCE_SCOPE_AGENT : HSA_FENCE_SCOPE_NONE;
-    else return fail(TL_ERR_INVALID, "engine_set_option: unknown option '" + n + "' (qmm3, qmm6, qmm7, gemm8, prefill_reduce_norm, attn_qkv_partials, lmhead_tile_max, gemm_fused_epilogue, aql_fences)");
-    return TL_OK;
+    else return fail(TL_ERR_INVALID, "engine_set_option: unknown option '" + n + "' (" + tl_engine_option_names() + ")");
+    return TL_OK;
+}
+
+extern "C" const char *tl_engine_prefill_route(const tl_engine *e) {
+    static thread_local std::string text;
+    if (!e) return "";
+    text = "fa_rows=" + std::to_string((int)e->prefill_route.fa_rows) + " qkv_post_reduce=" + std::to_string((int)e->prefill_route.qkv_post_reduce);
+    return text.c_str();
 }
 
 static void drop_plans(tl_engine *e) {
@@ -2399,28 +2417,64 @@
     return rc;
 }
 
-static int engine_paged_attention(tl_engine *e, int l, const uint16_t *q_t, const int32_t *block_row, const int32_t *ctx_dev, uint16_t *attn_t,
-                                  int n, int ctx_hint) {
+static int engine_paged_attention(tl_engine *e, int l, const uint16_t *q_t, const int32_t *block_row, const int32_t *ctx_dev, uint16_t *out,
+                                  int n, int ctx_hint, bool rows) {
     const tl_engine_config &c = e->cfg;
     const int D = c.head_dim, Hq = c.num_heads, Hkv = c.num_kv_heads;
-    if (e->kv_format == TL_KV_FP8_E4M3)
-        return tl_paged_attention_fp8(q_t, e->layer_k(l), e->layer_ks(l), e->layer_v(l), e->layer_vs(l), block_row, ctx_dev, attn_t, Hq, n, D,
-                                      c.num_pages, c.page_size, c.max_pages_per_seq, Hq, Hkv, 1.0f / sqrtf((float)D), 1, ctx_hint, e->attn_ws,
-                                      e->attn_ws_bytes, e->stream);
-    return tl_paged_attention(q_t, e->layer_k(l), e->layer_v(l), block_row, ctx_dev, attn_t, Hq, n, D, c.num_pages, c.page_size,
-                              c.max_pages_per_seq, Hq, Hkv, 1.0f / sqrtf((float)D), 1, ctx_hint, TL_BF16, e->attn_ws, e->attn_ws_bytes, e->stream);
+    const bool kv8 = e->kv_format == TL_KV_FP8_E4M3;
+    return tl_paged_attention_strided(q_t, e->layer_k(l), kv8 ? e->layer_ks(l) : nullptr, e->layer_v(l), kv8 ? e->layer_vs(l) : nullptr, block_row,
+                                      ctx_dev, out, Hq, n, D, c.num_pages, c.page_size, c.max_pages_per_seq, Hq, Hkv, 1.0f / sqrtf((float)D), 1,
+                                      ctx_hint, TL_BF16, e->attn_ws, e->attn_ws_bytes, rows ? (long)Hq * D : (long)D, rows ? (long)D : (long)n * D,
+                                      e->stream);
+}
+static bool qkv_post_takes_slices(int head_dim) { return head_dim == 128 || head_dim == 64; }
+static void launch_qkv_post_kernel(int head_dim, bool kv8, const QkvPostArgs &q, int n, hipStream_t st) {
+    const dim3 sliced(n, ceil_div(q.num_heads + 2 * q.num_kv_heads, 16));
+    switch (head_dim) {
+        case 128:
+            if (q.slices > 0) {
+                if (kv8) hipLaunchKernelGGL((qkv_post_kernel<8, true, true>), sliced, dim3(256), 0, st, q);
+                else hipLaunchKernelGGL((qkv_post_kernel<8, false, true>), sliced, dim3(256), 0, st, q);
+            } else if (kv8) hipLaunchKernelGGL((qkv_post_kernel<8, true>), dim3(n), dim3(256), 0, st, q);
+            else hipLaunchKernelGGL((qkv_post_kernel<8>), dim3(n), dim3(256), 0, st, q);
+            break;
+        case 64:
+            if (q.slices > 0) hipLaunchKernelGGL((qkv_post_kernel<4, false, true>), sliced, dim3(256), 0, st, q);
+            else hipLaunchKernelGGL((qkv_post_kernel<4>), dim3(n), dim3(256), 0, st, q);
+            break;
+        default: hipLaunchKernelGGL((qkv_post_kernel<2>), dim3(n), dim3(256), 0, st, q); break;
+    }
+}
+extern "C" int tl_qkv_post_rows(const void *partials_dev, int slices, void *qkv_rows_dev, const void *q_norm_dev, const void *k_norm_dev,
+                                void *q_t_dev, void *key_pages_dev, float *key_scales_dev, void *value_pages_dev, float *value_scales_dev,
+                                const int32_t *block_row_dev, int T, int start, int page_size, int max_pages, int num_heads, int num_kv_heads,
+                                int head_dim, float rope_theta, float eps, int fused, void *stream) {
+    TL_REQUIRE(partials_dev && q_norm_dev && k_norm_dev && q_t_dev && key_pages_dev && value_pages_dev && block_row_dev, "qkv_post_rows: null argument");
+    TL_REQUIRE(slices >= 1 && T >= 1 && start >= 0 && page_size > 0 && max_pages > 0 && num_heads > 0 && num_kv_heads > 0, "qkv_post_rows: bad shape");
+    TL_REQUIRE(head_dim == 128 || head_dim == 64 || head_dim == 32, "qkv_post_rows: head_dim is 128, 64 or 32");
+    TL_REQUIRE((key_scales_dev == nullptr) == (value_scales_dev == nullptr) && (!key_scales_dev || head_dim == 128), "qkv_post_rows: FP8 pages take both scale arrays and head_dim 128");
+    TL_REQUIRE((long)start + T <= (long)page_size * max_pages, "qkv_post_rows: the rows end past the block-table row");
+    TL_REQUIRE(fused ? qkv_post_takes_slices(head_dim) : qkv_rows_dev != nullptr, "qkv_post_rows: fused needs head_dim 128 or 64, unfused the qkv_rows buffer");
+    TL_REQUIRE(((uintptr_t)partials_dev | (uintptr_t)qkv_rows_dev | (uintptr_t)q_t_dev | (uintptr_t)key_pages_dev | (uintptr_t)value_pages_dev) % 16 == 0, "qkv_post_rows: buffers must be 16-byte aligned");
+    const size_t elements = (size_t)T * (num_heads + 2 * num_kv_heads) * head_dim;
+    hipStream_t st = (hipStream_t)stream;
+    QkvPostArgs q{};
+    if (!fused) TL_TRY(qmm_bf16_splitk_reduce((const uint16_t *)partials_dev, (uint16_t *)qkv_rows_dev, elements, slices, st));
+    q.qkv = fused ? (const uint16_t *)partials_dev : (const uint16_t *)qkv_rows_dev;
+    q.slices = fused ? slices : 0, q.plane = (long)elements;
+    q.q_norm_w = (const uint16_t *)q_norm_dev, q.k_norm_w = (const uint16_t *)k_norm_dev;
+    q.q_t = (uint16_t *)q_t_dev, q.key_pages = (uint16_t *)key_pages_dev, q.value_pages = (uint16_t *)value_pages_dev;
+    q.key_scales = key_scales_dev, q.value_scales = value_scales_dev;
+    q.block_row = block_row_dev, q.T = T, q.start = start, q.page_size = page_size, q.max_pages = max_pages;
+    q.num_heads = num_heads, q.num_kv_heads = num_kv_heads, q.eps = eps, q.rope_base = rope_theta;
+    launch_qkv_post_kernel(head_dim, key_scales_dev != nullptr, q, T, st);
+    TL_CHECK_LAUNCH("qkv_post_rows");
+    return TL_OK;
 }
 static void launch_qkv_post(tl_engine *e, int l, QkvPostArgs &q, int n) {
     q.key_scales = e->layer_ks(l);
     q.value_scales = e->layer_vs(l);
-    switch (e->cfg.head_dim) {
-        case 128:
-            if (e->kv_format == TL_KV_FP8_E4M3) hipLaunchKernelGGL((qkv_post_kernel<8, true>), dim3(n), dim3(256), 0, e->stream, q);
-            else hipLaunchKernelGGL((qkv_post_kernel<8>), dim3(n), dim3(256), 0, e->stream, q);
-            break;
-        case 64: hipLaunchKernelGGL((qkv_post_kernel<4>), dim3(n), dim3(256), 0, e->stream, q); break;
-        default: hipLaunchKernelGGL((qkv_post_kernel<2>), dim3(n), dim3(256), 0, e->stream, q); break;
-    }
+    launch_qkv_post_kernel(e->cfg.head_dim, e->kv_format == TL_KV_FP8_E4M3, q, n, e->stream);
 }
 
 struct PrefillSeq {
@@ -2481,20 +2535,29 @@
         return false;
     };
     bool x_normed = false;
+    const bool fa_rows = e->prefill_fa_rows && D == 128;
     for (int l = 0; l < c.num_layers; ++l) {
         const tl_layer_weights &w = e->layers[l];
         if (!x_normed) TL_TRY(tl_rms_norm(e->x, w.input_norm_dev, e->xn, total, c.hidden_size, c.rms_norm_eps, TL_BF16, e->stream));
         x_normed = false;
-        TL_TRY(engine_gemm(e->lin, proj(w.wqkv, e->xn, e->qkv, total)));
-        if (lora_on(l, tl_engine::LORA_QKV))
+        GemmKept kept;
+        const bool qkv_lora = lora_on(l, tl_engine::LORA_QKV);
+        TL_TRY(engine_gemm(e->lin, proj(w.wqkv, e->xn, e->qkv, total), nullptr,
+                           e->prefill_qkv_post_reduce && !qkv_lora && qkv_post_takes_slices(D) ? &kept : nullptr));
+        if (qkv_lora)
             TL_TRY(lora_group(e, l, tl_engine::LORA_QKV, e->lora_tiles_prefill, lora_tiles, total, e->xn, nullptr, TL_LORA_ADD, nullptr, e->qkv));
+        if (l == 0) e->prefill_route = {fa_rows, kept.slices > 0};
+        else e->prefill_route.qkv_post_reduce = e->prefill_route.qkv_post_reduce && kept.slices > 0;
         for (int i = 0; i < n_seqs; ++i) {
             const int n = seqs[i].len, start = seqs[i].start;
             const int32_t *block_row = e->block_table + (size_t)seqs[i].slot * c.max_pages_per_seq;
             uint16_t *q_t = e->q_t + (size_t)seqs[i].row0 * Hq * D;
             uint16_t *attn_t = e->attn_t + (size_t)seqs[i].row0 * Hq * D;
+            uint16_t *attn_rows = e->attn + (size_t)seqs[i].row0 * Hq * D;
             QkvPostArgs q{};
-            q.qkv = e->qkv + (size_t)seqs[i].row0 * (Hq + 2 * Hkv) * D;
+            q.qkv = (kept.slices > 0 ? kept.partials : e->qkv) + (size_t)seqs[i].row0 * (Hq + 2 * Hkv) * D;
+            q.slices = kept.slices;
+            q.plane = (long)kept.plane;
             q.q_norm_w = (const uint16_t *)w.q_norm_dev;
             q.k_norm_w = (const uint16_t *)w.k_norm_dev;
             q.q_t = q_t;
@@ -2511,10 +2574,11 @@
             q.rope_base = c.rope_theta;
             launch_qkv_post(e, l, q, n);
             TL_CHECK_LAUNCH("engine qkv_post");
-            TL_TRY(engine_paged_attention(e, l, q_t, block_row, e->scratch_ctx + i, attn_t, n, start + n));
-            const long items = (long)Hq * n * (D / 8);
-            hipLaunchKernelGGL(heads_to_rows_kernel, dim3(ceil_div(items, 256)), dim3(256), 0, e->stream, attn_t,
-                               e->attn + (size_t)seqs[i].row0 * Hq * D, Hq, n, D);
+            TL_TRY(engine_paged_attention(e, l, q_t, block_row, e->scratch_ctx + i, fa_rows ? attn_rows : attn_t, n, start + n, fa_rows));
+            if (!fa_rows) {
+                const long items = (long)Hq * n * (D / 8);
+                hipLaunchKernelGGL(heads_to_rows_kernel, dim3(ceil_div(items, 256)), dim3(256), 0, e->stream, attn_t, attn_rows, Hq, n, D);
+            }
         }
         bool h_normed = false;
         Proj po = proj(w.wo, e->attn, e->h, total);
diff --git a/tiny-llm_amd/csrc/engine_kernels.h b/tiny-llm_amd/csrc/engine_kernels.h
--- a/tiny-llm_amd/csrc/engine_kernels.h
+++ b/tiny-llm_amd/csrc/engine_kernels.h
@@ -56,11 +56,10 @@
 }
 
 template <int VD>
-__device__ __forceinline__ void head_norm_rope(const uint16_t *src, const uint16_t *w, int t, float eps,
-                                               const float (&cs)[VD], const float (&sn)[VD], float (&out)[VD]) {
+__device__ __forceinline__ void head_norm_rope_values(const float (&f)[VD], const uint16_t *w, int t, float eps,
+                                                      const float (&cs)[VD], const float (&sn)[VD], float (&out)[VD]) {
     constexpr int D = 16 * VD;
-    float f[VD], g[VD];
-    load_row<VD>(src + t * VD, f);
+    float g[VD];
     load_row<VD>(w + t * VD, g);
     float ss = 0.f;
 #pragma unroll
@@ -74,6 +73,39 @@
         const float r = (t < 8) ? (n * cs[i] - partner * sn[i]) : (n * cs[i] + partner * sn[i]);
         out[i] = bf16_round(r);
     }
+}
+
+template <int VD>
+__device__ __forceinline__ void head_norm_rope(const uint16_t *src, const uint16_t *w, int t, float eps,
+                                               const float (&cs)[VD], const float (&sn)[VD], float (&out)[VD]) {
+    float f[VD];
+    load_row<VD>(src + t * VD, f);
+    head_norm_rope_values<VD>(f, w, t, eps, cs, sn, out);
+}
+
+template <int VD>
+__device__ __forceinline__ void load_row_slices(const uint16_t *src, long plane, int slices, float (&f)[VD]) {
+    float sum[VD];
+#pragma unroll
+    for (int i = 0; i < VD; ++i) sum[i] = 0.f;
+    for (int p0 = 0; p0 < slices; p0 += 16) {
+        static_assert(VD == 8 || VD == 4 || VD == 2, "one vector load per slice");
+        using Raw = typename std::conditional<VD == 8, uint4, typename std::conditional<VD == 4, uint2, uint32_t>::type>::type;
+        Raw raw[16];
+#pragma unroll
+        for (int j = 0; j < 16; ++j) raw[j] = *reinterpret_cast<const Raw *>(src + (long)min(p0 + j, slices - 1) * plane);
+#pragma unroll
+        for (int j = 0; j < 16; ++j) {
+            if (p0 + j < slices) {
+                uint16_t e[VD];
+                *reinterpret_cast<Raw *>(e) = raw[j];
+#pragma unroll
+                for (int i = 0; i < VD; ++i) sum[i] += BF16::to_float(e[i]);
+            }
+        }
+    }
+#pragma unroll
+    for (int i = 0; i < VD; ++i) f[i] = bf16_round(sum[i]);
 }
 
 static __global__ __launch_bounds__(256) void rope_table_kernel(float2 *__restrict__ table, int max_pos, int half, float base) {
@@ -762,9 +794,11 @@
     int T, start, page_size, max_pages, num_heads, num_kv_heads;
     float eps, rope_base;
     float *key_scales, *value_scales;
+    int slices;
+    long plane;
 };
 
-template <int VD, bool KV8 = false>
+template <int VD, bool KV8 = false, bool QP = false>
 static __global__ __launch_bounds__(256) void qkv_post_kernel(const QkvPostArgs p) {
     static_assert(!KV8 || VD == 8, "FP8 pages: head dimension 128");
     constexpr int D = 16 * VD;
@@ -779,13 +813,15 @@
     const int lp = pos / p.page_size;
     const int slot = pos - lp * p.page_size;
     const int page_id = lp < p.max_pages ? p.block_row[lp] : -1;
-    for (int h = g; h < Hq + 2 * Hkv; h += 16) {
-        float v[VD];
+    for (int h = g + 16 * blockIdx.y; h < Hq + 2 * Hkv; h += 16 * gridDim.y) {
+        float v[VD], in[VD];
+        if constexpr (QP) load_row_slices<VD>(row + (long)h * D + t * VD, p.plane, p.slices, in);
+        else load_row<VD>(row + (long)h * D + t * VD, in);
         if (h < Hq) {
-            head_norm_rope<VD>(row + (long)h * D, p.q_norm_w, t, p.eps, cs, sn, v);
+            head_norm_rope_values<VD>(in, p.q_norm_w, t, p.eps, cs, sn, v);
             store_row<VD>(p.q_t + ((long)h * p.T + r) * D + t * VD, v);
         } else if (h < Hq + Hkv) {
-            head_norm_rope<VD>(row + (long)h * D, p.k_norm_w, t, p.eps, cs, sn, v);
+            head_norm_rope_values<VD>(in, p.k_norm_w, t, p.eps, cs, sn, v);
             const long prow = ((long)max(page_id, 0) * Hkv + (h - Hq)) * p.page_size + slot;
             if constexpr (KV8) {
                 u32x2 codes;
@@ -798,7 +834,8 @@
             } else if (page_id >= 0)
                 store_row<VD>(p.key_pages + prow * D + t * VD, v);
         } else {
-            load_row<VD>(row + (long)h * D + t * VD, v);
+#pragma unroll
+            for (int i = 0; i < VD; ++i) v[i] = in[i];
             const long prow = ((long)max(page_id, 0) * Hkv + (h - Hq - Hkv)) * p.page_size + slot;
             if constexpr (KV8) {
                 u32x2 codes;
diff --git a/tiny-llm_amd/csrc/qmm.hip b/tiny-llm_amd/csrc/qmm.hip
--- a/tiny-llm_amd/csrc/qmm.hip
+++ b/tiny-llm_amd/csrc/qmm.hip
@@ -510,6 +510,32 @@
     return TL_OK;
 }
 
+int qmm_bf16_keep_partials(const void *scales, const void *biases, const uint16_t *A, const uint32_t *b, int M, int N, int K, void *workspace,
+                           size_t workspace_bytes, hipStream_t st, int *slices, size_t *plane) {
+    if (M <= 8 || !slices || !plane) return fail(TL_ERR_INVALID, "qmm_bf16_keep_partials: for more than 8 rows");
+    const int split = split_k_policy(M, N, K);
+    *slices = split, *plane = (size_t)M * K;
+    if (split <= 1) return TL_OK;
+    if (!workspace || workspace_bytes < (size_t)split * M * K * 2)
+        return fail(TL_ERR_INVALID, "qmm_bf16_keep_partials: split-K workspace is missing or too small");
+    auto S = (const uint16_t *)scales;
+    auto Bi = (const uint16_t *)biases;
+    uint16_t *dst = (uint16_t *)workspace;
+    const int mt = mfma_mt(M), nw = mfma_nw(M, K), psize = N / split;
+    const size_t pstride = (size_t)M * K;
+    const dim3 grid(ceil_div(K, 32 * nw), ceil_div(M, 32 * mt), split), block(64 * nw);
+    if (nw == 8) hipLaunchKernelGGL((qmm_mfma_kernel<BF16, 4, 8>), grid, block, 0, st, S, Bi, A, b, dst, M, N, K, psize, pstride, nullptr, qmm_xcd_remap());
+    else if (mt == 1) hipLaunchKernelGGL((qmm_mfma_kernel<BF16, 1>), grid, block, 0, st, S, Bi, A, b, dst, M, N, K, psize, pstride, nullptr, qmm_xcd_remap());
+    else if (mt == 2) hipLaunchKernelGGL((qmm_mfma_kernel<BF16, 2>), grid, block, 0, st, S, Bi, A, b, dst, M, N, K, psize, pstride, nullptr, qmm_xcd_remap());
+    else hipLaunchKernelGGL((qmm_mfma_kernel<BF16, 4>), grid, block, 0, st, S, Bi, A, b, dst, M, N, K, psize, pstride, nullptr, qmm_xcd_remap());
+    return TL_OK;
+}
+
+int qmm_bf16_splitk_reduce(const uint16_t *partials, uint16_t *out, size_t elements, int slices, hipStream_t st) {
+    hipLaunchKernelGGL((splitk_reduce_kernel<BF16>), dim3(ceil_div(ceil_div(elements, 8), 256)), dim3(256), 0, st, partials, out, elements, slices);
+    return TL_OK;
+}
+
 template <typename TT>
 static int run_gather_qmv(const void *scales, const void *biases, const void *a, const uint32_t *b, const int32_t *expert_ids,
                           void *out, int M, int N, int K, int num_experts, hipStream_t st, int a_rows_div = 1) {
diff --git a/tiny-llm_amd/csrc/qmv.h b/tiny-llm_amd/csrc/qmv.h
--- a/tiny-llm_amd/csrc/qmv.h
+++ b/tiny-llm_amd/csrc/qmv.h
@@ -366,4 +366,7 @@
 int qmm_bf16_epilogue(const void *scales, const void *biases, const uint16_t *a, const uint32_t *b, uint16_t *out, int M, int N, int K,
                       int epi, const uint16_t *residual, void *workspace, size_t workspace_bytes, hipStream_t st, const uint16_t *norm_w = nullptr,
                       uint16_t *norm_out = nullptr, float norm_eps = 0.f, bool *norm_done = nullptr);
+int qmm_bf16_keep_partials(const void *scales, const void *biases, const uint16_t *a, const uint32_t *b, int M, int N, int K, void *workspace,
+                           size_t workspace_bytes, hipStream_t st, int *slices, size_t *plane);
+int qmm_bf16_splitk_reduce(const uint16_t *partials, uint16_t *out, size_t elements, int slices, hipStream_t st);
 }
diff --git a/tiny-llm_amd/extensions_hip/tiny_llm_ext_hip/__init__.py b/tiny-llm_amd/extensions_hip/tiny_llm_ext_hip/__init__.py
--- a/tiny-llm_amd/extensions_hip/tiny_llm_ext_hip/__init__.py
+++ b/tiny-llm_amd/extensions_hip/tiny_llm_ext_hip/__init__.py
@@ -55,6 +55,10 @@
     "tl_paged_attention_fp8": (
         _c_int,
         [_c_void_p] * 8 + [_c_int] * 8 + [_c_float, _c_int, _c_int, _c_void_p, _c_size_t, _c_void_p],
+    ),
+    "tl_paged_attention_strided": (
+        _c_int,
+        [_c_void_p] * 8 + [_c_int] * 8 + [_c_float, _c_int, _c_int, _c_int, _c_void_p, _c_size_t, ctypes.c_long, ctypes.c_long, _c_void_p],
     ),
 }
 
@@ -218,6 +222,9 @@
     "tl_decode_streaming_variant_compiled": (_c_int, [_c_int, _c_int]),
     "tl_decode_attention_plan": (_c_int, [_c_int, _c_int, _c_int, _c_int, _P(_c_int)]),
     "tl_engine_set_option": (_c_int, [_c_void_p, ctypes.c_char_p, _c_int]),
+    "tl_engine_option_names": (ctypes.c_char_p, []),
+    "tl_engine_prefill_route": (ctypes.c_char_p, [_c_void_p]),
+    "tl_qkv_post_rows": (_c_int, [_c_void_p, _c_int] + [_c_void_p] * 9 + [_c_int] * 7 + [_c_float, _c_float, _c_int, _c_void_p]),
     "tl_engine_destroy": (None, [_c_void_p]),
     "tl_engine_synchronize": (_c_int, [_c_void_p]),
     "tl_engine_begin": (_c_int, [_c_void_p, _c_int]),
@@ -1020,6 +1027,69 @@
     return out, {name: getattr(info, name) for name, _ in info._fields_}
 
 
+def paged_attention_rows(query: torch.Tensor, key_pages: torch.Tensor, value_pages: torch.Tensor, block_table: torch.Tensor,
+                         context_lens: torch.Tensor, scale: float = 1.0, is_causal: bool = False, *, num_kv_heads: int, num_heads: int,
+                         key_scales: torch.Tensor | None = None, value_scales: torch.Tensor | None = None,
+                         max_context_hint: int = 0) -> torch.Tensor:
+    fp8 = key_scales is not None
+    tensors = [query, key_pages, value_pages, block_table, context_lens] + ([key_scales, value_scales] if fp8 else [])
+    _require_gpu("paged_attention_rows", *tensors)
+    if not all(t.is_contiguous() for t in tensors) or block_table.dtype != torch.int32 or context_lens.dtype != torch.int32:
+        raise RuntimeError("paged_attention_rows: contiguous tensors, int32 block_table and context_lens")
+    if query.dim() != 3 or key_pages.dim() != 4 or key_pages.shape != value_pages.shape or query.shape[0] % num_heads != 0 \
+            or query.shape[0] // num_heads != block_table.shape[0] or block_table.shape[0] != context_lens.shape[0] \
+            or key_pages.shape[1] != num_kv_heads or key_pages.shape[3] != query.shape[2]:
+        raise RuntimeError("paged_attention_rows: q [B * H_q, L, D], pages [P, H_kv, page_size, D], block_table [B, max_pages], context_lens [B]")
+    if fp8 and (value_scales is None or key_pages.dtype != torch.uint8 or query.dtype != torch.bfloat16
+                or tuple(key_scales.shape) != tuple(key_pages.shape[:3]) or tuple(value_scales.shape) != tuple(key_pages.shape[:3])):
+        raise RuntimeError("paged_attention_rows: FP8 pages are uint8 with float32 scales [P, H_kv, page_size] and bfloat16 queries")
+    if not fp8 and (key_pages.dtype != query.dtype or value_pages.dtype != query.dtype):
+        raise RuntimeError("paged_attention_rows: q, key_pages and value_pages must have the same dtype")
+    N, L, D = query.shape
+    P, _, page_size, _ = key_pages.shape
+    max_pages = block_table.shape[1]
+    out = torch.empty((L, N * D), dtype=query.dtype, device=query.device)
+    ws_bytes = _lib.tl_paged_attention_workspace_bytes(N, L, D, page_size, max_pages, num_heads, num_kv_heads, int(max_context_hint))
+    ws = _workspace(ws_bytes, query.device)
+    _check(_lib.tl_paged_attention_strided(
+        _ptr(query), _ptr(key_pages), _ptr(key_scales) if fp8 else None, _ptr(value_pages), _ptr(value_scales) if fp8 else None,
+        _ptr(block_table), _ptr(context_lens), _ptr(out), N, L, D, P, page_size, max_pages, int(num_heads), int(num_kv_heads), float(scale),
+        int(bool(is_causal)), int(max_context_hint), _DTYPES[query.dtype], _ptr(ws) if ws is not None else None,
+        ws.numel() if ws is not None else 0, N * D, D, _stream()))
+    return out
+
+
+def qkv_post_rows(partials: torch.Tensor, q_norm: torch.Tensor, k_norm: torch.Tensor, key_pages: torch.Tensor, value_pages: torch.Tensor,
+                  block_row: torch.Tensor, start: int, *, num_heads: int, num_kv_heads: int, rope_theta: float, eps: float, fused: bool,
+                  key_scales: torch.Tensor | None = None, value_scales: torch.Tensor | None = None) -> torch.Tensor:
+    fp8 = key_scales is not None
+    tensors = [partials, q_norm, k_norm, key_pages, value_pages, block_row] + ([key_scales, value_scales] if fp8 else [])
+    _require_gpu("qkv_post_rows", *tensors)
+    P, Hkv, page_size, D = (int(x) for x in key_pages.shape)
+    if partials.dim() != 3 or partials.dtype != torch.bfloat16 or partials.shape[2] != (num_heads + 2 * num_kv_heads) * D or Hkv != num_kv_heads \
+            or tuple(value_pages.shape) != tuple(key_pages.shape) or block_row.dtype != torch.int32 or block_row.dim() != 1 \
+            or tuple(q_norm.shape) != (D,) or tuple(k_norm.shape) != (D,) or q_norm.dtype != torch.bfloat16 or k_norm.dtype != torch.bfloat16:
+        raise RuntimeError("qkv_post_rows: partials [S, T, (Hq + 2 Hkv) * D] bf16, pages [P, Hkv, page_size, D], block_row [max_pages] int32, norms [D] bf16")
+    if key_pages.dtype != (torch.uint8 if fp8 else torch.bfloat16) or value_pages.dtype != key_pages.dtype:
+        raise RuntimeError("qkv_post_rows: bf16 pages, or uint8 pages with scales")
+    if fp8 and (value_scales is None or tuple(key_scales.shape) != (P, Hkv, page_size) or tuple(value_scales.shape) != (P, Hkv, page_size)
+                or key_scales.dtype != torch.float32 or value_scales.dtype != torch.float32):
+        raise RuntimeError("qkv_post_rows: scales must be float32 [P, Hkv, page_size]")
+    if not all(t.is_contiguous() for t in tensors):
+        raise RuntimeError("qkv_post_rows: every tensor must be contiguous")
+    S, T, _ = (int(x) for x in partials.shape)
+    if int(block_row.max().item()) >= P or start < 0 or start + T > page_size * block_row.numel() \
+            or int(block_row[start // page_size:(start + T - 1) // page_size + 1].min().item()) < 0:
+        raise RuntimeError("qkv_post_rows: the rows' pages must be ids of the pool")
+    q_t = torch.empty((num_heads, T, D), dtype=torch.bfloat16, device=partials.device)
+    rows = None if fused else torch.empty((T, partials.shape[2]), dtype=torch.bfloat16, device=partials.device)
+    _check(_lib.tl_qkv_post_rows(
+        _ptr(partials), S, _ptr(rows) if rows is not None else None, _ptr(q_norm), _ptr(k_norm), _ptr(q_t), _ptr(key_pages),
+        _ptr(key_scales) if fp8 else None, _ptr(value_pages), _ptr(value_scales) if fp8 else None, _ptr(block_row), T, int(start), page_size,
+        int(block_row.numel()), int(num_heads), int(num_kv_heads), D, float(rope_theta), float(eps), int(bool(fused)), _stream()))
+    return q_t
+
+
 def paged_attention_waves(waves: int = 0) -> int:
     return int(_lib.tl_paged_attention_waves(int(waves)))
 
diff --git a/tiny-llm_amd/tiny_llm_hip/engine.py b/tiny-llm_amd/tiny_llm_hip/engine.py
--- a/tiny-llm_amd/tiny_llm_hip/engine.py
+++ b/tiny-llm_amd/tiny_llm_hip/engine.py
@@ -589,6 +589,10 @@
         c = _ext.TlStepCheck()
         _ext.check(_lib.tl_engine_check_step(self._h, batch or self.max_batch, ctypes.byref(c)))
         return {name: getattr(c, name) for name, _ in c._fields_}
+
+    def prefill_route(self) -> dict:
+        text = (_lib.tl_engine_prefill_route(self._h) or b"").decode()
+        return {k: int(v) for k, v in (item.split("=") for item in text.split())}
 
     def replay_route(self) -> str:
         return (_lib.tl_engine_replay_route(self._h) or b"").decode()
```

New measurement: 964.5 tokens/s. 0.99x the previous value.
